# panbanda/islands

Measured on AMD Instinct MI355X. Metric: queries/sec @ recall@10>=0.95, 10Mx768 ef=128, higher is better.
Workload: dtype f32; 1 GPU; 10000000 x 768 f32 rows resident in HBM (in-memory provider), hierarchical Gaussian mixture, graph by the harness (tools/synth.py::build_graph: k-means medoid levels flattened into one layer, diversified links, parent->child and reverse edges), deg<= 60 (mean 38.6), query batch 1024, k=10, ef=128, cosine; nodes=10000000, dim=768, query_batch=1024, k=10, ef=128, graph=harness, distinct_leaves=False, parallelism=single, searches_in_flight=32, distinct_batches=497, replayed_queries=1688

## Files before the change

### include/islands_amd.h

```cpp
#ifndef ISLANDS_AMD_H
#define ISLANDS_AMD_H

#include <stddef.h>
#include <stdint.h>

#ifdef __cplusplus
extern "C" {
#endif

#define ISL_ABI_VERSION 3

typedef int32_t isl_status;

enum {
  ISL_OK = 0,
  ISL_ERR_DIMENSION_MISMATCH = 1,
  ISL_ERR_EMPTY_COLLECTION = 2,
  ISL_ERR_INVALID_CONFIG = 3,
  ISL_ERR_INDEX_NOT_BUILT = 4,
  ISL_ERR_NODE_NOT_FOUND = 5,
  ISL_ERR_SERIALIZATION = 6,
  ISL_ERR_DESERIALIZATION = 7,
  ISL_ERR_IO = 8,
  ISL_ERR_HNSW = 9,
// ... 76 lines not shown
                            uint64_t n_new, uint64_t d, const uint64_t* levels, int32_t mem, uint64_t* first_id);
#define ISL_REMOVED UINT64_MAX
#define ISL_REMOVE_MAX_CANDIDATES 512u
isl_status isl_index_remove(isl_index* idx, const isl_build_options* opts, const uint64_t* ids, uint64_t n_ids,
                            uint64_t* out_remap , uint64_t* out_len );
isl_status isl_select_neighbors(const isl_index* idx, const isl_build_options* opts,
                                const uint64_t* base_ids, uint64_t nb, const uint64_t* cand_ids,
                                uint64_t pitch, const uint32_t* cand_cnt, uint64_t cap,
                                uint64_t* out_ids, uint32_t* out_cnt);

isl_status isl_index_from_bytes(const uint8_t* bytes, size_t len, isl_index** out);
isl_status isl_index_to_bytes(const isl_index* idx, uint8_t** out, size_t* len);
void isl_free_bytes(uint8_t* p);
void isl_index_free(isl_index* idx);

typedef struct isl_index_metadata {
  uint32_t version;
  uint64_t num_vectors;
  uint64_t dimension;
  int64_t created_at;
  int64_t updated_at;
  int32_t has_description;
  char description[256];
} isl_index_metadata;
void isl_index_metadata_new(uint64_t num_vectors, uint64_t dimension, int64_t now, isl_index_metadata* out);
isl_status isl_storage_write_metadata(const isl_index_metadata* meta, uint8_t** out, size_t* len);
isl_status isl_storage_read_metadata(const uint8_t* bytes, size_t len, isl_index_metadata* meta,
                                     size_t* consumed);
isl_status isl_index_save(const isl_index* idx, const char* path, const isl_index_metadata* meta);
isl_status isl_index_load(const char* path, isl_index** out, isl_index_metadata* meta);

uint64_t isl_index_len(const isl_index* idx);
int32_t isl_index_is_empty(const isl_index* idx);
int32_t isl_index_dimension(const isl_index* idx, uint64_t* dim);
uint64_t isl_index_storage_bytes(const isl_index* idx);
int32_t isl_index_is_recompute(const isl_index* idx);
int32_t isl_index_is_compact(const isl_index* idx);
isl_status isl_index_config(const isl_index* idx, isl_leann_config* out);
int32_t isl_index_entry_point(const isl_index* idx, uint64_t* entry);
uint64_t isl_index_max_level(const isl_index* idx);
int32_t isl_index_get_neighbors(const isl_index* idx, uint64_t node, const uint64_t** ptr,
                                size_t* len);

isl_status isl_index_upload(isl_index* idx, int32_t device);

isl_status isl_set_embeddings(isl_index* idx, const void* rows, uint64_t n, uint64_t d,
                              int32_t dtype, int32_t mem);

typedef struct isl_search_stats {
  uint64_t queries;
  uint64_t expansions;
  uint64_t edges;
  uint64_t evals;
  uint64_t pushes;
  uint64_t exact_path;
  uint64_t replayed;
  double kernel_ms;
  uint64_t encoded_nodes;
  uint64_t recompute_rounds;
  uint64_t allocations;
} isl_search_stats;

isl_status isl_index_prepare(isl_index* idx, uint64_t max_nq, uint64_t max_ef, uint64_t max_k,
                             int32_t lanes);

isl_status isl_search_batch(const isl_index* idx, const float* queries, uint64_t nq, uint64_t d,
                            uint64_t k, uint64_t ef, uint64_t* out_ids, float* out_dist,
                            uint32_t* out_count);
isl_status isl_search_batch_async(const isl_index* idx, const float* queries, uint64_t nq, uint64_t d,
                                  uint64_t k, uint64_t ef, uint64_t* out_ids, float* out_dist,
                                  uint32_t* out_count, uint64_t* token);
isl_status isl_search_batch_device(const isl_index* idx, const float* d_queries, uint64_t nq,
                                   uint64_t d, uint64_t k, uint64_t ef, uint64_t* d_out_ids,
                                   float* d_out_dist, uint32_t* d_out_count, void* stream);
isl_status isl_search_batch_device_async(const isl_index* idx, const float* d_queries, uint64_t nq,
                                         uint64_t d, uint64_t k, uint64_t ef, uint64_t* d_out_ids,
                                         float* d_out_dist, uint32_t* d_out_count, void* stream,
                                         uint64_t* token);
isl_status isl_search_wait_stats(const isl_index* idx, uint64_t token, isl_search_stats* stats);
isl_status isl_search_wait(const isl_index* idx, uint64_t token);
isl_status isl_search_stream_wait(const isl_index* idx, uint64_t token, void* stream);
isl_status isl_index_group_counters(const isl_index* idx, uint64_t* launches, uint64_t* shared_launches,
                                    uint64_t* shared_calls);
isl_status isl_search(const isl_index* idx, const float* query, uint64_t d, uint64_t k,
                      uint64_t* out_ids, float* out_dist, uint32_t* out_count);

isl_status isl_search_last_stats(const isl_index* idx, isl_search_stats* out);

#define ISL_MAX_ENTRY_SEEDS 65536ull
isl_status isl_index_select_entry_seeds(isl_index* idx, uint64_t count, uint64_t* out_ids, uint64_t* out_count);
isl_status isl_index_set_entry_seeds(isl_index* idx, const uint64_t* ids, uint64_t count);
isl_status isl_index_entry_seeds(const isl_index* idx, uint64_t* out, uint64_t cap, uint64_t* count);
isl_status isl_index_pick_entries(const isl_index* idx, const float* queries, uint64_t nq, uint64_t d,
                                  uint64_t* out_ids, int32_t mem, void* stream);

isl_status isl_distance(int32_t metric, const float* a, uint64_t na, const float* b, uint64_t nb,
                        float* out);
isl_status isl_distance_squared(int32_t metric, const float* a, uint64_t na, const float* b,
                                uint64_t nb, float* out);
isl_status isl_distance_batch(int32_t metric, const float* query, uint64_t d, const float* rows,
                              uint64_t n, uint64_t row_len, float* out, int32_t mem, int32_t device,
                              void* stream);
isl_status isl_normalize_rows(float* rows, uint64_t n, uint64_t d, int32_t mem, int32_t device,
                              void* stream);

isl_status isl_distance_matrix(int32_t metric, const float* queries, uint64_t nq, const float* rows,
                               uint64_t n, uint64_t d, float* out, int32_t mem, int32_t device,
                               void* stream);
isl_status isl_bruteforce_topk(int32_t metric, const float* queries, uint64_t nq, const float* rows,
                               uint64_t n, uint64_t d, uint64_t k, uint64_t* out_ids, float* out_dist,
                               uint32_t* out_count, int32_t mem, int32_t device, void* stream);

isl_status isl_merge_topk(uint64_t nlists, uint64_t nq, uint64_t k, const uint64_t* ids,
                          const float* scores, const uint32_t* counts, const uint64_t* id_base,
                          uint64_t top_k, uint64_t* out_ids, float* out_scores,
                          uint32_t* out_src, uint32_t* out_count, int32_t mem, int32_t device,
                          void* stream);
#define ISL_SHARD_POISON_COUNT 0xFFFFFFFFu
uint64_t isl_shard_record_bytes(uint64_t nq, uint64_t k);
isl_status isl_merge_topk_packed_async(uint64_t nlists, uint64_t nq, uint64_t k, const void* d_records,
                                       uint64_t list_stride, const uint64_t* d_id_base, uint64_t top_k,
                                       uint64_t* d_out_ids, float* d_out_scores, uint32_t* d_out_src,
                                       uint32_t* d_out_count, uint32_t* d_flags, int32_t device, void* stream);
#define ISL_SHARD_UNIQUE_ID_BYTES 128
typedef struct isl_shard_group isl_shard_group;
typedef int32_t (*isl_shard_allgather_fn)(void* user, const void* send, void* recv, uint64_t bytes);
isl_status isl_shard_unique_id(uint8_t id[ISL_SHARD_UNIQUE_ID_BYTES]);
isl_status isl_shard_group_create(int32_t device, int32_t world, int32_t rank,
                                  const uint8_t id[ISL_SHARD_UNIQUE_ID_BYTES], isl_shard_group** out);
isl_status isl_shard_group_create_host(int32_t device, int32_t world, int32_t rank,
                                       isl_shard_allgather_fn allgather, void* user, isl_shard_group** out);
isl_status isl_shard_group_info(const isl_shard_group* grp, int32_t* world, int32_t* rank, int32_t* comm_ranks,
                                int32_t* is_rccl);
void isl_shard_group_free(isl_shard_group* grp);

typedef struct isl_sharded_searcher isl_sharded_searcher;
isl_status isl_sharded_searcher_new(const isl_index* shard, isl_shard_group* grp, uint64_t n_total,
                                    const uint64_t* id_base, int32_t depth, isl_sharded_searcher** out);
void isl_sharded_searcher_free(isl_sharded_searcher* s);
isl_status isl_sharded_prepare(isl_sharded_searcher* s, uint64_t max_nq, uint64_t max_k, uint64_t max_ef);
isl_status isl_sharded_submit(isl_sharded_searcher* s, const float* d_queries, uint64_t nq, uint64_t d,
                              uint64_t k, uint64_t ef, void* stream, uint64_t* handle);
isl_status isl_sharded_result(isl_sharded_searcher* s, uint64_t handle, const uint64_t** d_ids,
                              const float** d_dist, const uint32_t** d_src, const uint32_t** d_count,
                              isl_search_stats* stats);
isl_status isl_sharded_search_batch(isl_sharded_searcher* s, const float* queries, uint64_t nq, uint64_t d,
                                    uint64_t k, uint64_t ef, uint64_t* out_ids, float* out_dist,
                                    uint32_t* out_src, uint32_t* out_count);
isl_status isl_sharded_flags(isl_sharded_searcher* s, uint32_t* flags);

isl_status isl_merge_service(uint64_t nlists, uint64_t nq, uint64_t k, const uint64_t* ids,
                             const float* distances, const uint32_t* counts,
                             const uint64_t* files_len, uint64_t top_k, uint64_t* out_ids,
                             float* out_scores, uint32_t* out_src, uint32_t* out_count,
                             int32_t mem, int32_t device, void* stream);

typedef struct isl_pq isl_pq;
isl_status isl_pq_new(uint64_t dimension, uint64_t m, uint64_t K, const float* codebooks,
                      int32_t metric, int32_t device, isl_pq** out);
void isl_pq_free(isl_pq* pq);
isl_status isl_pq_build_distance_tables(const isl_pq* pq, const float* queries, uint64_t nq,
                                        uint64_t d, float* tables, int32_t mem, void* stream);
isl_status isl_pq_table_distance(const isl_pq* pq, const float* tables, const uint16_t* codes,
                                 uint64_t n, float* out, int32_t mem, void* stream);
isl_status isl_pq_asymmetric_distance(const isl_pq* pq, const float* query, uint64_t d,
                                      const uint16_t* codes, uint64_t n, float* out, int32_t mem,
// ... 109 lines not shown
```

### include/islands_amd.hpp

```cpp
#pragma once

#include <cstdint>
#include <optional>
#include <stdexcept>
#include <string>
#include <utility>
#include <vector>

#include "islands_amd.h"

namespace islands::core {

struct CoreError : std::runtime_error {
  isl_status status;
  uint64_t expected, actual, node;
  CoreError(isl_status s, const std::string& msg, uint64_t e = 0, uint64_t a = 0, uint64_t n = 0)
      : std::runtime_error(msg), status(s), expected(e), actual(a), node(n) {}
  std::string kind() const { return isl_status_name(status); }
};

inline void check(isl_status s) {
  if (s != ISL_OK)
    throw CoreError(s, isl_last_error_message(), isl_last_error_expected(),
                    isl_last_error_actual(), isl_last_error_node());
// ... 117 lines not shown
    uint64_t first = 0;
    check(isl_index_insert(h_, &opts, n ? vectors.data() : nullptr, ISL_DTYPE_F32, n, d, levels, ISL_MEM_HOST, &first));
    return first;
  }
  uint64_t insert_bf16(const std::vector<uint16_t>& rows_bits, uint64_t n, uint64_t d,
                       const isl_build_options& opts = build_options(), const uint64_t* levels = nullptr) {
    uint64_t first = 0;
    check(isl_index_insert(h_, &opts, n ? rows_bits.data() : nullptr, ISL_DTYPE_BF16, n, d, levels, ISL_MEM_HOST,
                           &first));
    return first;
  }
  std::vector<uint64_t> remove(const std::vector<uint64_t>& ids, const isl_build_options& opts = build_options()) {
    std::vector<uint64_t> remap(len());
    check(isl_index_remove(h_, &opts, ids.empty() ? nullptr : ids.data(), ids.size(), remap.data(), nullptr));
    return remap;
  }
  std::vector<uint64_t> select_neighbors(uint64_t base, const std::vector<uint64_t>& candidates, uint64_t cap,
                                         const isl_build_options& opts = build_options()) const {
    std::vector<uint64_t> out(cap ? cap : 1);
    uint32_t cnt = (uint32_t)candidates.size(), n = 0;
    check(isl_select_neighbors(h_, &opts, &base, 1, candidates.data(), candidates.size(), &cnt, cap, out.data(), &n));
    out.resize(n);
    return out;
  }
  std::vector<uint8_t> to_bytes() const {
    uint8_t* p = nullptr;
    size_t n = 0;
    check(isl_index_to_bytes(h_, &p, &n));
    std::vector<uint8_t> out(p, p + n);
    isl_free_bytes(p);
    return out;
  }
  LeannIndex(LeannIndex&& o) noexcept : h_(o.h_) { o.h_ = nullptr; }
  LeannIndex& operator=(LeannIndex&& o) noexcept {
    if (this != &o) { isl_index_free(h_); h_ = o.h_; o.h_ = nullptr; }
    return *this;
  }
  LeannIndex(const LeannIndex&) = delete;
  LeannIndex& operator=(const LeannIndex&) = delete;
  ~LeannIndex() { isl_index_free(h_); }

  uint64_t len() const { return isl_index_len(h_); }
  bool is_empty() const { return isl_index_is_empty(h_) != 0; }
  std::optional<uint64_t> dimension() const {
    uint64_t d = 0;
    return isl_index_dimension(h_, &d) ? std::optional<uint64_t>(d) : std::nullopt;
  }
  uint64_t storage_bytes() const { return isl_index_storage_bytes(h_); }
  bool is_recompute() const { return isl_index_is_recompute(h_) != 0; }
  bool is_compact() const { return isl_index_is_compact(h_) != 0; }
  LeannConfig config() const { LeannConfig c; check(isl_index_config(h_, &c)); return c; }

  void upload(int32_t device = 0) { check(isl_index_upload(h_, device)); }
  void attach(const InMemoryEmbeddingProvider& p) {
    check(isl_set_embeddings(h_, p.embeddings.data(), p.len(), p.dim, ISL_DTYPE_F32, ISL_MEM_HOST));
  }
  void attach_recompute(isl_encoder* enc, const std::vector<uint16_t>& tokens, uint64_t n, uint64_t L,
                        bool normalize = true, bool keep_rows = false) {
    check(isl_set_recompute_provider(h_, enc, tokens.data(), nullptr, n, L, normalize ? 1 : 0,
                                     keep_rows ? 1 : 0, ISL_MEM_HOST));
  }
  std::vector<uint64_t> select_entry_seeds(uint64_t count) {
    std::vector<uint64_t> ids(count < len() ? count : len());
    uint64_t n = 0;
    check(isl_index_select_entry_seeds(h_, count, ids.data(), &n));
    ids.resize(n);
    return ids;
  }
  void set_entry_seeds(const std::vector<uint64_t>& ids) { check(isl_index_set_entry_seeds(h_, ids.data(), ids.size())); }
  std::vector<uint64_t> entry_seeds() const {
    uint64_t n = 0;
    check(isl_index_entry_seeds(h_, nullptr, 0, &n));
    std::vector<uint64_t> ids(n);
    check(isl_index_entry_seeds(h_, ids.data(), n, &n));
    return ids;
  }
  std::vector<uint64_t> pick_entries(const std::vector<float>& queries, uint64_t nq) const {
    std::vector<uint64_t> ids(nq);
    check(isl_index_pick_entries(h_, queries.data(), nq, nq ? queries.size() / nq : 0, ids.data(), ISL_MEM_HOST, nullptr));
    return ids;
  }
  void prepare(uint64_t max_nq, uint64_t max_ef, uint64_t max_k = 10, int32_t lanes = 8) {
    check(isl_index_prepare(h_, max_nq, max_ef, max_k, lanes));
  }
  std::vector<std::pair<uint64_t, float>> search(const std::vector<float>& query, uint64_t k) const {
    return search_with_params(query, k, config().ef_search);
  }
  std::vector<std::pair<uint64_t, float>> search_with_params(const std::vector<float>& query,
                                                             uint64_t k, uint64_t ef) const {
    std::vector<uint64_t> ids(k ? k : 1);
    std::vector<float> dist(k ? k : 1);
    uint32_t cnt = 0;
    check(isl_search_batch(h_, query.data(), 1, query.size(), k, ef, ids.data(), dist.data(), &cnt));
    std::vector<std::pair<uint64_t, float>> out;
    for (uint32_t i = 0; i < cnt; i++) out.emplace_back(ids[i], dist[i]);
    return out;
  }
  void attach_pq_codes(const isl_pq* pq, const std::vector<uint16_t>& codes, uint64_t n) {
    check(isl_index_set_pq_codes(h_, pq, codes.data(), n, ISL_MEM_HOST));
  }
  std::vector<std::pair<uint64_t, float>> search_two_level(const std::vector<float>& query, uint64_t k,
                                                           uint64_t ef, float rerank_ratio) const {
    std::vector<uint64_t> ids(k ? k : 1);
    std::vector<float> dist(k ? k : 1);
    uint32_t cnt = 0;
    check(isl_search_two_level_batch(h_, query.data(), 1, query.size(), k, ef, rerank_ratio, ids.data(),
                                     dist.data(), &cnt));
    std::vector<std::pair<uint64_t, float>> out;
    for (uint32_t i = 0; i < cnt; i++) out.emplace_back(ids[i], dist[i]);
    return out;
  }
  isl_index* handle() const { return h_; }

 private:
  explicit LeannIndex(std::nullptr_t) {}
  isl_index* h_ = nullptr;
};

struct SearchResult {
  uint64_t id = 0;
  float score = 0.f;
  std::optional<std::vector<float>> vector;
  std::optional<std::string> text;
  float to_similarity() const { return 1.0f / (1.0f + score); }
};

struct SearchConfig {
  uint64_t top_k = 10, ef = 100;
  bool include_vectors = false, include_metadata = true;
  std::optional<float> min_similarity;
  static SearchConfig fast(uint64_t k) { SearchConfig c; c.top_k = k; c.ef = k * 2; return c; }
  static SearchConfig accurate(uint64_t k) { SearchConfig c; c.top_k = k; c.ef = k * 10; return c; }
};

class HnswGraph {
 public:
  HnswGraph(const std::vector<float>& vectors, uint64_t dim,
            const std::vector<std::vector<std::vector<uint64_t>>>& layers,
            const std::vector<uint64_t>& levels, std::optional<uint64_t> entry_point, uint64_t max_level,
            uint64_t m = 16, uint64_t m0 = 32, uint64_t ef_construction = 200,
            DistanceMetric metric = DistanceMetric::Cosine, int32_t device = 0)
      : vectors_(vectors), dim_(dim) {
    const uint64_t n = levels.size();
    std::vector<std::vector<uint64_t>> offs(layers.size()), adjs(layers.size());
    std::vector<const uint64_t*> po, pa;
    for (size_t L = 0; L < layers.size(); L++) {
      offs[L].assign(1, 0);
      for (uint64_t i = 0; i < n; i++) {
        adjs[L].insert(adjs[L].end(), layers[L][i].begin(), layers[L][i].end());
        offs[L].push_back(adjs[L].size());
      }
      if (adjs[L].empty()) adjs[L].push_back(0);
      po.push_back(offs[L].data());
      pa.push_back(adjs[L].data());
    }
    check(isl_hnsw_from_layers(m, m0, ef_construction, (int32_t)metric, n, dim, layers.size(), po.data(),
                               pa.data(), n ? levels.data() : nullptr, entry_point ? 1 : 0,
                               entry_point.value_or(0), max_level, n ? vectors.data() : nullptr, device, &h_));
  }
  static HnswGraph from_bytes(const std::vector<uint8_t>& bytes, int32_t device = 0) {
    HnswGraph g;
    check(isl_hnsw_from_bytes(bytes.data(), bytes.size(), device, &g.h_));
    return g;
  }
  static HnswGraph build(const std::vector<float>& vectors, uint64_t dim, const isl_hnsw_config* cfg = nullptr,
                         const std::vector<uint64_t>& levels = {}, uint64_t level_seed = 0,
// ... 176 lines not shown
```

### islands_amd/__init__.py

```python
from __future__ import annotations

import ctypes as C
import enum
import os
from dataclasses import dataclass, field

import numpy as np

from . import _ffi
from ._ffi import BertConfigC, BuildOptionsC, IndexMetadataC, LeannConfigC, SearchStatsC, u64

__all__ = [
    "CoreError", "DistanceMetric", "PruningStrategy", "LeannConfig", "CsrGraph",
    "InMemoryEmbeddingProvider", "LeannIndex", "ProductQuantizer", "SearchResult",
    "batch_calculate", "calculate", "calculate_squared", "normalize_rows", "distance_matrix",
    "bruteforce_topk", "merge_topk", "merge_service",
    "device_count", "HnswGraph", "SearchConfig", "Searcher", "MultiIndexSearcher",
    "mean_pool_normalize", "service_search", "BertConfig", "CandleEmbedder", "IndexMetadata",
]

MEM_HOST, MEM_DEVICE = 0, 1
SELECT_REFERENCE, SELECT_DIVERSE = 0, 1
_SELECT_RULES = {"reference": SELECT_REFERENCE, "diverse": SELECT_DIVERSE}
REMOVED = 0xFFFFFFFFFFFFFFFF
# ... 618 lines not shown
            q = q.reshape(1, -1)
        nq, d = q.shape
        ids = np.zeros((nq, max(k, 1)), dtype=np.uint64)
        dist = np.zeros((nq, max(k, 1)), dtype=np.float32)
        cnt = np.zeros(nq, dtype=np.uint32)
        _check(_ffi.lib().isl_search_two_level_batch(self._h, _ptr(q), nq, d, k, ef,
                                                     C.c_float(rerank_ratio), _ptr(ids), _ptr(dist),
                                                     _ptr(cnt)))
        return ids[:, :k], dist[:, :k], cnt

    def search_two_level_batch_device(self, d_queries_ptr: int, nq: int, d: int, k: int, ef: int,
                                      rerank_ratio: float, d_ids_ptr: int, d_dist_ptr: int,
                                      d_count_ptr: int, stream: int = 0):
        _check(_ffi.lib().isl_search_two_level_batch_device(
            self._h, C.c_void_p(d_queries_ptr), nq, d, k, ef, C.c_float(rerank_ratio),
            C.c_void_p(d_ids_ptr), C.c_void_p(d_dist_ptr), C.c_void_p(d_count_ptr),
            C.c_void_p(stream)))

    def search_two_level_batch_device_async(self, d_queries_ptr: int, nq: int, d: int, k: int, ef: int,
                                            rerank_ratio: float, d_ids_ptr: int, d_dist_ptr: int,
                                            d_count_ptr: int, stream: int = 0) -> int:
        tok = C.c_uint64()
        _check(_ffi.lib().isl_search_two_level_batch_device_async(
            self._h, C.c_void_p(d_queries_ptr), nq, d, k, ef, C.c_float(rerank_ratio),
            C.c_void_p(d_ids_ptr), C.c_void_p(d_dist_ptr), C.c_void_p(d_count_ptr),
            C.c_void_p(stream), C.byref(tok)))
        return int(tok.value)

    def search_batch_device(self, d_queries_ptr: int, nq: int, d: int, k: int, ef: int,
                            d_ids_ptr: int, d_dist_ptr: int, d_count_ptr: int, stream: int = 0):
        _check(_ffi.lib().isl_search_batch_device(
            self._h, C.c_void_p(d_queries_ptr), nq, d, k, ef, C.c_void_p(d_ids_ptr),
            C.c_void_p(d_dist_ptr), C.c_void_p(d_count_ptr), C.c_void_p(stream)))

    def search_batch_device_async(self, d_queries_ptr: int, nq: int, d: int, k: int, ef: int,
                                  d_ids_ptr: int, d_dist_ptr: int, d_count_ptr: int,
                                  stream: int = 0) -> int:
        tok = C.c_uint64()
        _check(_ffi.lib().isl_search_batch_device_async(
            self._h, C.c_void_p(d_queries_ptr), nq, d, k, ef, C.c_void_p(d_ids_ptr),
            C.c_void_p(d_dist_ptr), C.c_void_p(d_count_ptr), C.c_void_p(stream), C.byref(tok)))
        return int(tok.value)

    def wait(self, token: int):
        try:
            _check(_ffi.lib().isl_search_wait(self._h, token))
        finally:
            out = self._pending.pop(token, None)
        return out

    def wait_stats(self, token: int) -> dict:
        s = SearchStatsC()
        try:
            _check(_ffi.lib().isl_search_wait_stats(self._h, token, C.byref(s)))
        finally:
            self._pending.pop(token, None)
        return {f: getattr(s, f) for f, _ in SearchStatsC._fields_}

    def prepare(self, max_nq: int, max_ef: int, max_k: int = 10, lanes: int = 8) -> "LeannIndex":
        _check(_ffi.lib().isl_index_prepare(self._h, max_nq, max_ef, max_k, lanes))
        return self

    def search_batch_async(self, queries, k: int, ef: int, out=None) -> int:
        q = _f32(queries)
        if q.ndim == 1:
            q = q.reshape(1, -1)
        nq, d = q.shape
        if out is None:
            out = (np.zeros((nq, max(k, 1)), dtype=np.uint64), np.zeros((nq, max(k, 1)), dtype=np.float32),
                   np.zeros(nq, dtype=np.uint32))
        ids, dist, cnt = out
        tok = C.c_uint64()
        _check(_ffi.lib().isl_search_batch_async(self._h, _ptr(q), nq, d, k, ef, _ptr(ids), _ptr(dist),
                                                 _ptr(cnt), C.byref(tok)))
        t = int(tok.value)
        if t:
            self._pending[t] = out
        return t

    def last_stats(self) -> dict:
        s = SearchStatsC()
        _check(_ffi.lib().isl_search_last_stats(self._h, C.byref(s)))
        return {f: getattr(s, f) for f, _ in SearchStatsC._fields_}


def merge_topk(ids, scores, counts, top_k: int, id_base=None, device: int = 0):
    ids = np.ascontiguousarray(ids, dtype=np.uint64)
    scores = _f32(scores)
    counts = np.ascontiguousarray(counts, dtype=np.uint32)
    nl, nq, k = ids.shape
    base = None if id_base is None else np.ascontiguousarray(id_base, dtype=np.uint64)
    oi = np.zeros((nq, max(top_k, 1)), dtype=np.uint64)
    osc = np.zeros((nq, max(top_k, 1)), dtype=np.float32)
    osrc = np.zeros((nq, max(top_k, 1)), dtype=np.uint32)
    oc = np.zeros(nq, dtype=np.uint32)
    _check(_ffi.lib().isl_merge_topk(nl, nq, k, _ptr(ids), _ptr(scores), _ptr(counts),
                                     None if base is None else _ptr(base), top_k, _ptr(oi),
                                     _ptr(osc), _ptr(osrc), _ptr(oc), MEM_HOST, device, None))
    return oi[:, :top_k], osc[:, :top_k], osrc[:, :top_k], oc


def merge_service(ids, distances, counts, top_k: int, files_len=None, device: int = 0):
    ids = np.ascontiguousarray(ids, dtype=np.uint64)
    distances = _f32(distances)
    counts = np.ascontiguousarray(counts, dtype=np.uint32)
    nl, nq, k = ids.shape
    fl = None if files_len is None else np.ascontiguousarray(files_len, dtype=np.uint64)
    oi = np.zeros((nq, max(top_k, 1)), dtype=np.uint64)
    osc = np.zeros((nq, max(top_k, 1)), dtype=np.float32)
    osrc = np.zeros((nq, max(top_k, 1)), dtype=np.uint32)
    oc = np.zeros(nq, dtype=np.uint32)
    _check(_ffi.lib().isl_merge_service(nl, nq, k, _ptr(ids), _ptr(distances), _ptr(counts),
                                        None if fl is None else _ptr(fl), top_k, _ptr(oi),
                                        _ptr(osc), _ptr(osrc), _ptr(oc), MEM_HOST, device, None))
    return oi[:, :top_k], osc[:, :top_k], osrc[:, :top_k], oc


class ProductQuantizer:

    def __init__(self, dimension: int, codebooks, metric=DistanceMetric.Euclidean, device: int = 0):
        cb = _f32(codebooks)
        m, K, dsub = cb.shape
        if m * dsub != dimension:
            raise CoreError(3, f"Invalid configuration: dimension {dimension} must be divisible by "
                               f"num_subquantizers {m}")
        self.dimension, self.m, self.K, self.dsub = dimension, m, K, dsub
        self._h = C.c_void_p()
        _check(_ffi.lib().isl_pq_new(dimension, m, K, _ptr(cb), int(metric), device,
                                     C.byref(self._h)))

    def __del__(self):
        h = getattr(self, "_h", None)
        if h:
            try:
                _ffi.lib().isl_pq_free(h)
            except Exception:
                pass
            self._h = None

    def num_subquantizers(self) -> int:
        return self.m

    def bytes_per_vector(self) -> int:
        return self.m if self.K <= 256 else self.m * 2

    def compression_ratio(self) -> float:
        return float(np.float32(self.dimension * 4) / np.float32(self.bytes_per_vector()))

    def build_distance_tables(self, queries) -> np.ndarray:
        q = _f32(queries)
        single = q.ndim == 1
        if single:
            q = q.reshape(1, -1)
        nq, d = q.shape
        t = np.zeros((nq, self.m, self.K), dtype=np.float32)
        _check(_ffi.lib().isl_pq_build_distance_tables(self._h, _ptr(q), nq, d, _ptr(t), MEM_HOST,
                                                       None))
        return t[0] if single else t

    def table_distance(self, tables, codes) -> np.ndarray:
        t = _f32(tables)
        c = np.ascontiguousarray(codes, dtype=np.uint16).reshape(-1, self.m)
        out = np.zeros(c.shape[0], dtype=np.float32)
        _check(_ffi.lib().isl_pq_table_distance(self._h, _ptr(t), _ptr(c), c.shape[0], _ptr(out),
                                                MEM_HOST, None))
        return out
# ... 487 lines not shown
```

### islands_amd/_ffi.py

```python
from __future__ import annotations

import ctypes as C
import os

os.environ.setdefault("GPU_MAX_HW_QUEUES", "32")

_HERE = os.path.dirname(os.path.abspath(__file__))
LIB_PATH = os.environ.get("ISL_AMD_LIB") or os.path.join(_HERE, "lib", "libislands_amd.so")

u64, u32, i32, f32 = C.c_uint64, C.c_uint32, C.c_int32, C.c_float
P = C.POINTER


class LeannConfigC(C.Structure):
    _fields_ = [
        ("m", u64), ("m0", u64), ("ef_construction", u64), ("ml", C.c_double),
        ("max_layers", u64), ("metric", u32), ("ef_search", u64), ("beam_width", u64),
        ("prune_ratio", f32), ("pruning_strategy", u32), ("high_degree_pruning", C.c_uint8),
        ("hub_percentile", f32), ("is_compact", C.c_uint8), ("is_recompute", C.c_uint8),
    ]


class BertConfigC(C.Structure):
    _fields_ = [("vocab_size", u32), ("hidden", u32), ("layers", u32), ("heads", u32),
                ("intermediate", u32), ("max_position", u32), ("type_vocab", u32),
                ("layer_norm_eps", f32), ("gelu_tanh", u32)]


class IndexMetadataC(C.Structure):
    _fields_ = [("version", u32), ("num_vectors", u64), ("dimension", u64), ("created_at", C.c_int64),
                ("updated_at", C.c_int64), ("has_description", i32), ("description", C.c_char * 256)]


class SearchStatsC(C.Structure):
    _fields_ = [("queries", u64), ("expansions", u64), ("edges", u64), ("evals", u64),
                ("pushes", u64), ("exact_path", u64), ("replayed", u64), ("kernel_ms", C.c_double),
                ("encoded_nodes", u64), ("recompute_rounds", u64), ("allocations", u64)]


class BuildOptionsC(C.Structure):
    _fields_ = [("struct_size", u32), ("select_rule", u32), ("alpha", f32), ("keep_pruned", u32),
                ("batch", u64)]


class HnswConfigC(C.Structure):
    _fields_ = [("m", u64), ("m0", u64), ("ef_construction", u64), ("ml", C.c_double), ("metric", u32),
                ("max_layers", u64)]


SIGNATURES = {
    "isl_last_error_message": (C.c_char_p, []),
    "isl_last_error_expected": (u64, []),
    "isl_last_error_actual": (u64, []),
    "isl_last_error_node": (u64, []),
    "isl_status_name": (C.c_char_p, [i32]),
    "isl_abi_version": (u32, []),
    "isl_device_count": (i32, []),
    "isl_leann_config_paper_default": (None, [P(LeannConfigC)]),
    "isl_leann_config_fast": (None, [P(LeannConfigC)]),
    "isl_leann_config_accurate": (None, [P(LeannConfigC)]),
    "isl_leann_config_validate": (i32, [P(LeannConfigC)]),
    "isl_index_new": (i32, [P(LeannConfigC), P(C.c_void_p)]),
    "isl_index_from_csr": (i32, [P(LeannConfigC), u64, C.c_void_p, C.c_void_p, C.c_void_p,
                                 C.c_void_p, i32, u64, u64, i32, u64, P(C.c_void_p)]),
    "isl_index_from_device_csr": (i32, [P(LeannConfigC), i32, u64, C.c_void_p, C.c_void_p, i32,
                                        u64, i32, u64, P(C.c_void_p)]),
    "isl_index_from_bytes": (i32, [C.c_void_p, C.c_size_t, P(C.c_void_p)]),
    "isl_index_to_bytes": (i32, [C.c_void_p, P(C.c_void_p), P(C.c_size_t)]),
    "isl_free_bytes": (None, [C.c_void_p]),
    "isl_index_free": (None, [C.c_void_p]),
    "isl_index_len": (u64, [C.c_void_p]),
    "isl_index_is_empty": (i32, [C.c_void_p]),
    "isl_index_dimension": (i32, [C.c_void_p, P(u64)]),
    "isl_index_storage_bytes": (u64, [C.c_void_p]),
    "isl_index_is_recompute": (i32, [C.c_void_p]),
    "isl_index_is_compact": (i32, [C.c_void_p]),
    "isl_index_config": (i32, [C.c_void_p, P(LeannConfigC)]),
    "isl_index_entry_point": (i32, [C.c_void_p, P(u64)]),
    "isl_index_max_level": (u64, [C.c_void_p]),
    "isl_index_get_neighbors": (i32, [C.c_void_p, u64, P(P(u64)), P(C.c_size_t)]),
    "isl_index_upload": (i32, [C.c_void_p, i32]),
    "isl_set_embeddings": (i32, [C.c_void_p, C.c_void_p, u64, u64, i32, i32]),
    "isl_search_batch": (i32, [C.c_void_p, C.c_void_p, u64, u64, u64, u64, C.c_void_p,
                               C.c_void_p, C.c_void_p]),
    "isl_hnsw_from_bytes": (i32, [C.c_void_p, C.c_size_t, i32, P(C.c_void_p)]),
    "isl_distance_matrix_bf16": (i32, [i32, C.c_void_p, u64, C.c_void_p, u64, u64, C.c_void_p, i32, i32,
                                       C.c_void_p]),
    "isl_index_set_pq_codes": (i32, [C.c_void_p, C.c_void_p, C.c_void_p, u64, i32]),
    "isl_search_two_level_batch": (i32, [C.c_void_p, C.c_void_p, u64, u64, u64, u64, C.c_float,
                                         C.c_void_p, C.c_void_p, C.c_void_p]),
    "isl_search_two_level_batch_device": (i32, [C.c_void_p, C.c_void_p, u64, u64, u64, u64,
                                                C.c_float, C.c_void_p, C.c_void_p, C.c_void_p,
                                                C.c_void_p]),
    "isl_search_two_level_batch_device_async": (i32, [C.c_void_p, C.c_void_p, u64, u64, u64, u64,
                                                      C.c_float, C.c_void_p, C.c_void_p, C.c_void_p,
                                                      C.c_void_p, P(u64)]),
    "isl_search_batch_device": (i32, [C.c_void_p, C.c_void_p, u64, u64, u64, u64, C.c_void_p,
                                      C.c_void_p, C.c_void_p, C.c_void_p]),
    "isl_search_batch_device_async": (i32, [C.c_void_p, C.c_void_p, u64, u64, u64, u64, C.c_void_p,
                                            C.c_void_p, C.c_void_p, C.c_void_p, P(u64)]),
    "isl_search_wait": (i32, [C.c_void_p, u64]),
    "isl_search_stream_wait": (i32, [C.c_void_p, u64, C.c_void_p]),
    "isl_index_group_counters": (i32, [C.c_void_p, P(u64), P(u64), P(u64)]),
    "isl_shard_record_bytes": (u64, [u64, u64]),
    "isl_merge_topk_packed_async": (i32, [u64, u64, u64, C.c_void_p, u64, C.c_void_p, u64, C.c_void_p, C.c_void_p,
                                          C.c_void_p, C.c_void_p, C.c_void_p, i32, C.c_void_p]),
    "isl_shard_unique_id": (i32, [C.c_void_p]),
    "isl_shard_group_create": (i32, [i32, i32, i32, C.c_void_p, P(C.c_void_p)]),
    "isl_shard_group_create_host": (i32, [i32, i32, i32, C.c_void_p, C.c_void_p, P(C.c_void_p)]),
    "isl_shard_group_info": (i32, [C.c_void_p, P(i32), P(i32), P(i32), P(i32)]),
    "isl_shard_group_free": (None, [C.c_void_p]),
    "isl_sharded_searcher_new": (i32, [C.c_void_p, C.c_void_p, u64, C.c_void_p, i32, P(C.c_void_p)]),
    "isl_sharded_searcher_free": (None, [C.c_void_p]),
    "isl_sharded_prepare": (i32, [C.c_void_p, u64, u64, u64]),
    "isl_sharded_submit": (i32, [C.c_void_p, C.c_void_p, u64, u64, u64, u64, C.c_void_p, P(u64)]),
    "isl_sharded_result": (i32, [C.c_void_p, u64, P(C.c_void_p), P(C.c_void_p), P(C.c_void_p), P(C.c_void_p),
                                 P(SearchStatsC)]),
    "isl_sharded_search_batch": (i32, [C.c_void_p, C.c_void_p, u64, u64, u64, u64, C.c_void_p, C.c_void_p,
                                       C.c_void_p, C.c_void_p]),
    "isl_sharded_flags": (i32, [C.c_void_p, P(u32)]),
    "isl_search_wait_stats": (i32, [C.c_void_p, u64, P(SearchStatsC)]),
    "isl_search_batch_async": (i32, [C.c_void_p, C.c_void_p, u64, u64, u64, u64, C.c_void_p,
                                     C.c_void_p, C.c_void_p, P(u64)]),
    "isl_index_prepare": (i32, [C.c_void_p, u64, u64, u64, i32]),
    "isl_search": (i32, [C.c_void_p, C.c_void_p, u64, u64, C.c_void_p, C.c_void_p, C.c_void_p]),
    "isl_search_last_stats": (i32, [C.c_void_p, P(SearchStatsC)]),
    "isl_distance": (i32, [i32, C.c_void_p, u64, C.c_void_p, u64, P(f32)]),
    "isl_distance_squared": (i32, [i32, C.c_void_p, u64, C.c_void_p, u64, P(f32)]),
    "isl_distance_batch": (i32, [i32, C.c_void_p, u64, C.c_void_p, u64, u64, C.c_void_p, i32, i32,
                                 C.c_void_p]),
    "isl_normalize_rows": (i32, [C.c_void_p, u64, u64, i32, i32, C.c_void_p]),
    "isl_distance_matrix": (i32, [i32, C.c_void_p, u64, C.c_void_p, u64, u64, C.c_void_p, i32, i32,
                                  C.c_void_p]),
    "isl_bruteforce_topk": (i32, [i32, C.c_void_p, u64, C.c_void_p, u64, u64, u64, C.c_void_p,
                                  C.c_void_p, C.c_void_p, i32, i32, C.c_void_p]),
    "isl_row_sumsq_bf16": (i32, [C.c_void_p, u64, u64, C.c_void_p, i32, i32, C.c_void_p]),
    "isl_distance_matrix_bf16_norms": (i32, [i32, C.c_void_p, u64, C.c_void_p, u64, u64, C.c_void_p, C.c_void_p,
                                             C.c_void_p, i32, i32, C.c_void_p]),
    "isl_distance_matrix_bf16_enqueue": (i32, [i32, C.c_void_p, u64, C.c_void_p, u64, u64, C.c_void_p, C.c_void_p,
                                               C.c_void_p, i32, C.c_void_p]),
    "isl_bruteforce_topk_bf16": (i32, [i32, C.c_void_p, u64, C.c_void_p, u64, u64, u64, C.c_void_p,
                                       C.c_void_p, C.c_void_p, i32, i32, C.c_void_p]),
    "isl_merge_topk": (i32, [u64, u64, u64, C.c_void_p, C.c_void_p, C.c_void_p, C.c_void_p, u64,
                             C.c_void_p, C.c_void_p, C.c_void_p, C.c_void_p, i32, i32,
                             C.c_void_p]),
    "isl_merge_service": (i32, [u64, u64, u64, C.c_void_p, C.c_void_p, C.c_void_p, C.c_void_p, u64,
                             C.c_void_p, C.c_void_p, C.c_void_p, C.c_void_p, i32, i32,
                             C.c_void_p]),
    "isl_index_build": (i32, [P(LeannConfigC), C.c_void_p, u64, u64, C.c_void_p, u64, i32, i32,
                              P(C.c_void_p)]),
    "isl_build_options_default": (None, [P(BuildOptionsC)]),
    "isl_index_build_ex": (i32, [P(LeannConfigC), P(BuildOptionsC), C.c_void_p, u64, u64, C.c_void_p, i32, i32,
                                 P(C.c_void_p)]),
    "isl_index_build_rows": (i32, [P(LeannConfigC), P(BuildOptionsC), C.c_void_p, i32, u64, u64, C.c_void_p, i32, i32,
                                   P(C.c_void_p)]),
    "isl_select_neighbors": (i32, [C.c_void_p, P(BuildOptionsC), C.c_void_p, u64, C.c_void_p, u64, C.c_void_p,
                                   u64, C.c_void_p, C.c_void_p]),
    "isl_index_select_entry_seeds": (i32, [C.c_void_p, u64, C.c_void_p, P(u64)]),
    "isl_index_set_entry_seeds": (i32, [C.c_void_p, C.c_void_p, u64]),
    "isl_index_entry_seeds": (i32, [C.c_void_p, C.c_void_p, u64, P(u64)]),
    "isl_index_pick_entries": (i32, [C.c_void_p, C.c_void_p, u64, u64, C.c_void_p, i32, C.c_void_p]),
    "isl_index_metadata_new": (None, [u64, u64, C.c_int64, P(IndexMetadataC)]),
    "isl_storage_write_metadata": (i32, [P(IndexMetadataC), P(C.c_void_p), P(C.c_size_t)]),
    "isl_storage_read_metadata": (i32, [C.c_void_p, C.c_size_t, P(IndexMetadataC), P(C.c_size_t)]),
    "isl_index_save": (i32, [C.c_void_p, C.c_char_p, P(IndexMetadataC)]),
    "isl_index_load": (i32, [C.c_char_p, P(C.c_void_p), P(IndexMetadataC)]),
    "isl_encoder_new": (i32, [P(BertConfigC), i32, P(C.c_void_p)]),
    "isl_encoder_free": (None, [C.c_void_p]),
    "isl_encoder_set_weight": (i32, [C.c_void_p, C.c_char_p, C.c_void_p, u64, i32]),
    "isl_encoder_set_precision": (i32, [C.c_void_p, i32]),
    "isl_encoder_forward": (i32, [C.c_void_p, C.c_void_p, C.c_void_p, C.c_void_p, u64, u64,
                                  C.c_void_p, i32, C.c_void_p]),
    "isl_encoder_embed": (i32, [C.c_void_p, C.c_void_p, C.c_void_p, C.c_void_p, u64, u64, i32,
                                C.c_void_p, i32, C.c_void_p]),
    "isl_set_recompute_provider": (i32, [C.c_void_p, C.c_void_p, C.c_void_p, C.c_void_p, u64, u64,
                                         i32, i32, i32]),
    "isl_index_set_recompute_cache_rows": (i32, [C.c_void_p, u64]),
    "isl_index_recompute_cache_bytes": (u64, [C.c_void_p]),
    "isl_mean_pool_normalize": (i32, [C.c_void_p, C.c_void_p, u64, u64, u64, i32, C.c_void_p, i32,
                                      i32, C.c_void_p]),
    "isl_hnsw_from_layers": (i32, [u64, u64, u64, i32, u64, u64, u64, C.c_void_p, C.c_void_p,
                                   C.c_void_p, i32, u64, u64, C.c_void_p, i32, P(C.c_void_p)]),
    "isl_hnsw_free": (None, [C.c_void_p]),
    "isl_hnsw_len": (u64, [C.c_void_p]),
    "isl_hnsw_last_stats": (i32, [C.c_void_p, P(SearchStatsC)]),
    "isl_hnsw_search_batch": (i32, [C.c_void_p, C.c_void_p, u64, u64, u64, u64, C.c_void_p,
# ... 49 lines not shown
```

### islands_amd/csrc/common.hpp

```cpp
#pragma once

#include <hip/hip_runtime.h>

#include <algorithm>
#include <cstdarg>
#include <cstdint>
#include <cstdlib>
#include <cstdio>
#include <cstring>
#include <atomic>
#include <chrono>
#include <mutex>
#include <string>
#include <thread>
#include <type_traits>
#include <vector>

#include "../../include/islands_amd.h"
#include "device_buffer.hpp"
#include "row_table.hpp"

namespace isl {

struct ErrorRecord {
  std::string message;
  uint64_t expected = 0, actual = 0, node = 0;
};
ErrorRecord& last_error();
isl_status fail(isl_status st, const char* fmt, ...);
isl_status fail_dim(uint64_t expected, uint64_t actual);
isl_status fail_node(uint64_t node);

#define ISL_HIP(expr)                                                                   \
  do {                                                                                  \
    hipError_t _e = (expr);                                                             \
    if (_e != hipSuccess)                                                               \
      return ::isl::fail(ISL_ERR_DEVICE, "%s failed: %s (%s:%d)", #expr,                \
                         hipGetErrorString(_e), __FILE__, __LINE__);                    \
  } while (0)

#define ISL_TRY(expr)            \
  do {                           \
    isl_status _s = (expr);      \
    if (_s != ISL_OK) return _s; \
  } while (0)

template <class F>
void by_metric(uint32_t metric, F&& f) {
  switch (metric) {
    case ISL_METRIC_COSINE: f(std::integral_constant<int, ISL_METRIC_COSINE>{}); break;
    case ISL_METRIC_EUCLIDEAN: f(std::integral_constant<int, ISL_METRIC_EUCLIDEAN>{}); break;
    case ISL_METRIC_DOT: f(std::integral_constant<int, ISL_METRIC_DOT>{}); break;
    default: f(std::integral_constant<int, ISL_METRIC_MANHATTAN>{}); break;
  }
}

isl_status use_device(int32_t device);
int device_cu_count(int32_t device);

struct SearchWorkspace {
  uint32_t slots = 0;
  uint32_t ovf_bits = 0;
  DeviceBuffer<uint32_t> ovf_tab;
  DeviceBuffer<uint32_t> status;
  DeviceBuffer<uint64_t> payload;
  DeviceBuffer<uint32_t> ctr;
  DeviceBuffer<uint32_t> ticket;
  DeviceBuffer<uint32_t> redo;
  DeviceBuffer<uint32_t> replay;
  DeviceBuffer<uint32_t> qsel;
  DeviceBuffer<uint32_t> qsel_h;
  DeviceBuffer<uint64_t> plog;
  DeviceBuffer<float> q_stage;
  DeviceBuffer<uint64_t> ids_stage;
  DeviceBuffer<float> dist_stage;
  DeviceBuffer<uint32_t> count_stage;
  PinnedBuffer<float> h_q;
  PinnedBuffer<uint64_t> h_ids;
  PinnedBuffer<float> h_dist;
  PinnedBuffer<uint32_t> h_count;
  hipStream_t stream = nullptr;
  hipEvent_t ev0 = nullptr, ev1 = nullptr, ev_in = nullptr, ev_done = nullptr;
  bool busy = false;
  bool waiting = false;
  bool enqueued = false;
  bool ticket_clean = false;
  bool publish_results = false;
  uint64_t token = 0;
  uint64_t nq_inflight = 0, k_inflight = 0;
  uint32_t ef_inflight = 0;
  bool fast_inflight = false;
  hipStream_t st_inflight = nullptr;
  uint64_t* u_ids = nullptr;
  float* u_dist = nullptr;
  uint32_t* u_count = nullptr;
  PinnedBuffer<uint32_t> h_status;
  PinnedBuffer<uint32_t> h_ctr;
  PinnedBuffer<uint32_t> h_head;
  DeviceBuffer<uint64_t> d_prof;
  DeviceBuffer<uint64_t> d_tline;
  DeviceBuffer<uint32_t> q_entry;
  DeviceBuffer<float> co_q;
  DeviceBuffer<uint64_t> co_ids;
  DeviceBuffer<float> co_dist;
  DeviceBuffer<uint32_t> co_cnt;
  DeviceBuffer<uint32_t> miss;
  DeviceBuffer<uint32_t> uniq;
  DeviceBuffer<uint32_t> uniq_count;
  uint64_t miss_cap = 0;
  uint64_t pref_cap = 0;
  DeviceBuffer<uint32_t> qstate;
  DeviceBuffer<uint32_t> qflag;
  DeviceBuffer<uint32_t> qlist;
  PinnedBuffer<uint32_t> h_qlist;
  DeviceBuffer<uint32_t> uslots;
  DeviceBuffer<uint32_t> xslot;
  PinnedBuffer<uint32_t> h_xlist;
  DeviceBuffer<float> tl_tables;
  std::thread* worker = nullptr;
  bool threaded = false;
  isl_status worker_status = ISL_OK;
  ErrorRecord worker_error;
  uint64_t alloc_events = 0;
  uint64_t alloc_mark = 0;
  isl_search_stats stats{};
  bool grp = false;
  SearchWorkspace* grp_launch = nullptr;
  uint32_t grp_offset = 0;
  hipEvent_t grp_ready = nullptr;
  uint64_t grp_allocs = 0;
  bool grp_failed = false;
  isl_status grp_status = ISL_OK;
  ErrorRecord grp_error;
  int32_t pool_lane = -1;
  bool union_launch = false;
  PinnedBuffer<uint64_t> h_members;
  DeviceBuffer<uint32_t> grp_scratch;
};

constexpr int kSearchLanes = 32;

int hw_queues_at_load();
constexpr int kGroupBelowQueues = 8;
struct GroupSwitches { bool off; uint32_t cap, room; };
inline GroupSwitches group_switches() {
  auto num = [](const char* name) -> uint32_t {
    const char* e = getenv(name);
    const long long v = e ? atoll(e) : 0;
    return v > 0 ? (uint32_t)std::min<long long>(v, 0x7FFFFFFF) : 0u;
  };
  const char* off = getenv("ISL_NO_GROUP");
  const bool is_off = (off && *off) ? strcmp(off, "0") != 0 : hw_queues_at_load() >= kGroupBelowQueues;
  return GroupSwitches{is_off, num("ISL_GROUP_CAP"), num("ISL_GROUP_ROOM")};
}
struct GroupState;

struct ExactPool {
  uint32_t slots = 0;
  uint64_t cand_cap = 0;
  DeviceBuffer<float> cand_d;
  DeviceBuffer<uint32_t> cand_id;
  DeviceBuffer<uint32_t> vis_bits;
  uint64_t vis_words = 0;
  DeviceBuffer<uint32_t> ulist;
  uint32_t ulist_cap = 0;
  DeviceBuffer<uint32_t> locks;
  DeviceBuffer<uint32_t> xstate;
  uint32_t xstate_words = 0;
};

}

struct isl_pq {
  uint64_t dimension = 0, m = 0, K = 0, dsub = 0, cstride = 0;
  int32_t metric = ISL_METRIC_EUCLIDEAN;
  int32_t device = 0;
  isl::DeviceBuffer<float> d_codebooks;
};

struct isl_index {
  isl_leann_config cfg{};
  bool host_csr_valid = true;
  std::vector<uint64_t> node_offsets{0};
  std::vector<uint64_t> neighbors;
  std::vector<uint64_t> levels;
  std::vector<uint64_t> degree_counts;
  bool has_entry = false;
  uint64_t entry_point = 0;
  uint64_t max_level = 0;
  uint64_t num_nodes = 0;
  bool has_dimension = false;
  uint64_t dimension = 0;

  int32_t device = -1;
  isl::DeviceBuffer<uint64_t> d_off;
  isl::DeviceBuffer<uint32_t> d_adj;
  uint64_t nnz = 0;
  uint32_t max_degree = 0;
  mutable std::atomic<uint64_t> evals_hint{0};
  isl::RowTable rows;
  uint64_t nvec = 0;

  isl::EntrySeeds seeds;

  uint32_t* d_ell = nullptr;
  uint32_t* d_ell_deg = nullptr;
  uint32_t ell_w = 0;
  isl::DeviceBuffer<uint32_t> ell_copy, ell_deg_copy;

  uint32_t* build_q_entry = nullptr;
  uint32_t* build_q_evals = nullptr;

  struct isl_encoder* enc = nullptr;
  isl::DeviceBuffer<uint16_t> d_tokens;
  isl::DeviceBuffer<uint16_t> d_lens;
  uint32_t tok_L = 0;
  isl::DeviceBuffer<uint32_t> d_slot_of;
  isl::DeviceBuffer<uint32_t> d_owner;
  isl::DeviceBuffer<uint32_t> d_stamp;
  isl::DeviceBuffer<uint32_t> d_slab_head;
  mutable uint32_t round_no = 1;
  bool recompute = false, keep_rows = false;
  int32_t enc_normalize = 1;

  bool is_hnsw = false;
  uint64_t hnsw_layers = 0;
  isl::DeviceBuffer<const uint64_t*> d_layer_off;
  isl::DeviceBuffer<const uint32_t*> d_layer_adj;
  std::vector<isl::DeviceBuffer<unsigned char>> hnsw_owned;

  const isl_pq* pq = nullptr;
  isl::DeviceBuffer<uint16_t> d_codes;
  uint64_t ncodes = 0;

  mutable std::mutex mu;
  mutable std::mutex recompute_mu;
  struct RecJoin {
    std::mutex mu;
    std::mutex leader;
    std::vector<void*> waiting;
  };
  mutable RecJoin rec_join;
  mutable isl::SearchWorkspace ws[isl::kSearchLanes];
  mutable isl::ExactPool pool;
  mutable uint64_t next_token = 1;
  const isl::GroupSwitches group_sw = isl::group_switches();
  mutable std::mutex group_mu;
  mutable isl::GroupState* group = nullptr;
};

struct isl_hnsw {
  isl_index* core = nullptr;
  uint64_t m = 0, m0 = 0, ef_construction = 0;
  uint64_t dim = 0;
  double ml = 0.0;
  uint64_t max_layers = 16;
  int32_t device = 0;
  std::vector<const uint64_t*> layer_off;
  std::vector<const uint32_t*> layer_adj;
  mutable std::mutex host_mu;
  mutable bool host_valid = false;
  mutable std::vector<std::vector<uint64_t>> h_off;
  mutable std::vector<std::vector<uint64_t>> h_adj;
};

namespace isl {
isl_status search_device_sync(const isl_index* idx, const float* d_queries, uint64_t nq, uint64_t d,
                              uint64_t k, uint64_t ef, uint64_t* d_ids, float* d_dist,
                              uint32_t* d_count, hipStream_t stream);
isl_status poison_failed_queries(const isl_index* idx, uint64_t token, uint32_t* d_counts, uint64_t nq, hipStream_t stream);
isl_status materialise_host_csr(const isl_index* idx);
isl_status set_grown_embeddings(isl_index* idx, const isl_index* old, const void* rows, int32_t dtype, uint64_t n_new,
                                uint64_t d, int32_t mem);
isl_status pq_launch_tables(const isl_pq* pq, const float* d_queries, uint64_t nq, float* d_tables,
                            hipStream_t st);
isl_status launch_entry_pick(const isl_index* idx, const float* d_queries, uint64_t nq, uint32_t* q_entry,
                             uint32_t* q_evals, unsigned long long* packed, uint32_t* status, uint64_t* d_out_ids,
                             hipStream_t st);
isl_status env_entry_seeds(isl_index* idx);
void free_workspace(SearchWorkspace& ws);
void free_exact_pool(ExactPool& pool);
bool any_lane_busy(const isl_index* idx);
void join_lane_workers(const isl_index* idx);
void free_group_state(isl_index* idx);
isl_status ensure_padded_adjacency(isl_index* idx);
isl_status hnsw_config_validate(uint64_t m, uint64_t m0, uint64_t ef_construction, int64_t metric);
isl_status attach_upper_layers(isl_hnsw* h, const std::vector<const uint64_t*>& offs,
                               const std::vector<const uint32_t*>& adjs);
}
```

### islands_amd/csrc/search.hip

```cpp
#include "search_geometry.hpp"
#include "search_internal.hpp"

using namespace isl_lane;

namespace {

__global__ void fill_u32_kernel(uint32_t* p, uint64_t n, uint32_t v) {
  uint64_t i = (uint64_t)blockIdx.x * blockDim.x + threadIdx.x;
  uint64_t stride = (uint64_t)gridDim.x * blockDim.x;
  for (; i < n; i += stride) p[i] = v;
}

struct PublishParams {
  const uint32_t* src[6];
  uint32_t* dst[6];
  uint32_t words[6];
  uint32_t ticket_seg;
};
__global__ void publish_kernel(PublishParams pp) {
  const uint32_t seg = blockIdx.y;
  const uint32_t n = pp.words[seg];
  const uint32_t* __restrict__ src = pp.src[seg];
  uint32_t* __restrict__ dst = pp.dst[seg];
  for (uint32_t i = blockIdx.x * blockDim.x + threadIdx.x; i < n; i += gridDim.x * blockDim.x) {
    dst[i] = src[i];
    if (seg == pp.ticket_seg) const_cast<uint32_t*>(src)[i] = 0u;
  }
}
__global__ void copy_u128_kernel(const uint4* __restrict__ src, uint4* __restrict__ dst, uint64_t n) {
  for (uint64_t i = (uint64_t)blockIdx.x * blockDim.x + threadIdx.x; i < n; i += (uint64_t)gridDim.x * blockDim.x)
    dst[i] = src[i];
}
__global__ void copy_u32_kernel(const uint32_t* __restrict__ src, uint32_t* __restrict__ dst, uint64_t n) {
  for (uint64_t i = (uint64_t)blockIdx.x * blockDim.x + threadIdx.x; i < n; i += (uint64_t)gridDim.x * blockDim.x)
    dst[i] = src[i];
}

__global__ void seed_redo_kernel(const uint32_t* __restrict__ list, uint32_t n, uint32_t* __restrict__ redo,
                                 uint32_t* __restrict__ ticket) {
  for (uint32_t i = threadIdx.x; i < n; i += blockDim.x) redo[i] = list[i];
  if (threadIdx.x == 0) ticket[1] = n;
}

constexpr uint32_t kExactSlots = 32;
constexpr uint32_t kOvfBits = 15;


hipStream_t pool_stream(int32_t device, uint32_t lane, bool* created) {
  static std::mutex mu;
  static hipStream_t pool[64][32];
  static const uint32_t size = [] {
    const char* e = getenv("ISL_MAX_STREAMS");
    const int v = e ? atoi(e) : 16;
    return (uint32_t)std::min(std::max(v, 1), 32);
  }();
  *created = false;
  if (device < 0 || device >= 64) return nullptr;
  std::lock_guard<std::mutex> lock(mu);
  hipStream_t& st = pool[device][lane % size];
  if (!st) {
    if (hipStreamCreateWithFlags(&st, hipStreamNonBlocking) != hipSuccess) { (void)hipGetLastError(); st = nullptr; }
    else *created = true;
  }
  return st;
}

}

isl_status isl_lane::ensure_lane_stream(const isl_index* idx, isl::SearchWorkspace& ws) {
  if (ws.stream) return ISL_OK;
  bool created = false;
  hipStream_t st = pool_stream(idx->device, ws.pool_lane >= 0 ? (uint32_t)ws.pool_lane : (uint32_t)(&ws - idx->ws), &created);
  if (!st) return isl::fail(ISL_ERR_DEVICE, "hipStreamCreate failed for a search lane");
  if (created) ws.alloc_events++;
  if (!ws.ev_done) { ISL_HIP(hipEventCreateWithFlags(&ws.ev_done, hipEventDisableTiming)); ws.alloc_events++; }
  if (!ws.ev0) { ISL_HIP(hipEventCreate(&ws.ev0)); ws.alloc_events++; }
  if (!ws.ev1) { ISL_HIP(hipEventCreate(&ws.ev1)); ws.alloc_events++; }
  if (!ws.ev_in) { ISL_HIP(hipEventCreateWithFlags(&ws.ev_in, hipEventDisableTiming)); ws.alloc_events++; }
  if (!ws.ticket) {
    ISL_TRY(ws.ticket.reserve(16, &ws.alloc_events));
    ws.ticket_clean = false;
  }
  ISL_TRY(ws.h_head.reserve(16, &ws.alloc_events));
  ws.stream = st;
  return ISL_OK;
}

void isl_lane::copy_words(const uint32_t* src, uint32_t* dst, uint64_t n, uint32_t grid, uint32_t block, hipStream_t st) {
  hipLaunchKernelGGL(copy_u32_kernel, dim3(grid), dim3(block), 0, st, src, dst, n);
}

isl_status isl_lane::prepare_workspace(const isl_index* idx, isl::SearchWorkspace& ws, uint32_t nq, uint32_t slots,
                                       uint32_t plog_cap) {
  ISL_TRY(ensure_lane_stream(idx, ws));
  uint64_t* const ev = &ws.alloc_events;
  const uint64_t cap = nq < 1024 ? 1024 : nq;
  ISL_TRY(ws.h_status.reserve(cap, ev));
  ISL_TRY(ws.h_ctr.reserve(cap * 4, ev));
  if (ws.slots < slots || !ws.ovf_tab) {
    ws.ovf_tab.reset();
    ws.slots = 0;
    static const uint32_t ovf_bits_cfg = [] {
      const char* e = getenv("ISL_OVF_BITS");
      const int v = e ? atoi(e) : (int)kOvfBits;
      return (uint32_t)std::min(15, std::max(10, v));
    }();
    ws.ovf_bits = ovf_bits_cfg;
    uint64_t n = (uint64_t)slots << ovf_bits_cfg;
    ISL_TRY(ws.ovf_tab.reserve(n, ev));
    hipLaunchKernelGGL(fill_u32_kernel, dim3(2048), dim3(256), 0, ws.stream, ws.ovf_tab, n, EMPTY);
    ISL_HIP(hipGetLastError());
    ISL_HIP(hipStreamSynchronize(ws.stream));
    ws.slots = slots;
  }
  ISL_TRY(ws.status.reserve(cap, ev));
  ISL_TRY(ws.payload.reserve(cap, ev));
  ISL_TRY(ws.ctr.reserve(cap * 4, ev));
  ISL_TRY(ws.redo.reserve(cap, ev));
  ISL_TRY(ws.replay.reserve(cap, ev));
  ISL_TRY(ws.qsel.reserve(cap, ev));
  ISL_TRY(ws.qsel_h.reserve(cap, ev));
  return ws.plog.reserve(ws.status.capacity() * plog_cap, ev);
}

namespace {

isl_status prepare_host_staging(isl::SearchWorkspace& ws, uint64_t nq, uint64_t d, uint64_t k) {
  uint64_t* const ev = &ws.alloc_events;
  ISL_TRY(ws.q_stage.reserve(nq * d, ev));
  ISL_TRY(ws.h_q.reserve(nq * d, ev));
  const uint64_t slots = nq * std::max<uint64_t>(k, 1);
  ISL_TRY(ws.ids_stage.reserve(slots, ev));
  ISL_TRY(ws.dist_stage.reserve(slots, ev));
  ISL_TRY(ws.count_stage.reserve(slots, ev));
  ISL_TRY(ws.h_ids.reserve(slots, ev));
  ISL_TRY(ws.h_dist.reserve(slots, ev));
  return ws.h_count.reserve(slots, ev);
}

}

isl_status isl_lane::ensure_pool(const isl_index* idx, isl::SearchWorkspace& ws) {
  isl::ExactPool& pl = idx->pool;
  if (pl.slots) return ISL_OK;
  uint64_t max_id = std::max(idx->num_nodes, idx->nvec);
  pl.vis_words = (max_id + 31) / 32 + 1;
  pl.cand_cap = std::min<uint64_t>(max_id + 1, 1ull << 21);
  pl.ulist_cap = std::max<uint32_t>(idx->max_degree, 64);
  isl_status st = ISL_OK;
  uint64_t* const ev = &ws.alloc_events;
  pl.xstate_words = 16 + 2 * (kMaxExactEf + 1);
  if ((st = pl.cand_d.reserve(kExactSlots * pl.cand_cap, ev)) == ISL_OK &&
      (st = pl.cand_id.reserve(kExactSlots * pl.cand_cap, ev)) == ISL_OK &&
      (st = pl.vis_bits.reserve(kExactSlots * pl.vis_words, ev)) == ISL_OK &&
      (st = pl.ulist.reserve((uint64_t)kExactSlots * pl.ulist_cap, ev)) == ISL_OK &&
      (st = pl.locks.reserve(kExactSlots, ev)) == ISL_OK &&
      (st = pl.xstate.reserve((uint64_t)kExactSlots * pl.xstate_words, ev)) == ISL_OK) {
    if (hipMemset(pl.locks, 0, (size_t)kExactSlots * 4) == hipSuccess) {
      pl.slots = kExactSlots;
      return ISL_OK;
    }
    st = isl::fail(ISL_ERR_DEVICE, "hipMemset failed for the exact-kernel pool");
  }
  isl::free_exact_pool(pl);
  return st;
}

namespace {

__global__ void pad_rows_kernel(const uint64_t* __restrict__ off, const uint32_t* __restrict__ adj, uint64_t n,
                                uint32_t W, uint32_t* __restrict__ ell, uint32_t* __restrict__ deg) {
  const uint64_t row = (uint64_t)blockIdx.x * 4 + (threadIdx.x >> 6);
  const uint32_t lane = threadIdx.x & 63;
  if (row >= n) return;
  const uint64_t o0 = off[row];
  const uint32_t d = (uint32_t)(off[row + 1] - o0);
  for (uint32_t i = lane; i < W; i += 64) ell[row * W + i] = i < d ? adj[o0 + i] : EMPTY;
  if (lane == 0) deg[row] = d;
}

isl_status publish(isl::SearchWorkspace& ws, uint64_t nq, uint64_t k, hipStream_t st) {
  PublishParams pp{};
  uint32_t n = 0;
  auto seg = [&](const void* src, void* dst, uint64_t words) {
    pp.src[n] = (const uint32_t*)src; pp.dst[n] = (uint32_t*)dst; pp.words[n] = (uint32_t)words; ++n;
  };
  seg(ws.status, ws.h_status, nq);
  seg(ws.ctr, ws.h_ctr, nq * 4);
  pp.ticket_seg = n;
  seg(ws.ticket, ws.h_head, 16);
  if (ws.publish_results) {
    seg(ws.count_stage, ws.h_count, nq);
    if (k) {
      seg(ws.ids_stage, ws.h_ids, nq * k * 2);
      seg(ws.dist_stage, ws.h_dist, nq * k);
    }
  }
  hipLaunchKernelGGL(publish_kernel, dim3(16, n), dim3(256), 0, st, pp);
  ISL_HIP(hipGetLastError());
  ws.ticket_clean = true;
  return ISL_OK;
}


void launch_fast(const isl_launch::FastKernel& k, uint32_t grid, size_t lds, hipStream_t st, const SearchParams& p) {
  switch (k.S) {
    case 1: isl_launch::launch_fast_segments<1>(k, grid, lds, st, &p); break;
    case 2: isl_launch::launch_fast_segments<2>(k, grid, lds, st, &p); break;
    case 4: isl_launch::launch_fast_segments<4>(k, grid, lds, st, &p); break;
    default: isl_launch::launch_fast_segments<8>(k, grid, lds, st, &p); break;
  }
}

isl_status search_enqueue_impl(const isl_index* idx, isl::SearchWorkspace& ws, const SearchCall& c,
                               const RoundPlan& plan, bool warm) {
  const uint64_t nq = c.nq, d = c.d, k = c.k;
  if (nq > 0x7FFFFFFFull) return isl::fail(ISL_ERR_INVALID_ARGUMENT, "too many queries");
  const TwoLevelCall tl_call{c.ratio, plan.window_scale};
  const TwoLevelCall* tl = c.two_level ? &tl_call : nullptr;
  CallGeometry cg;
  ISL_TRY(call_geometry(idx, d, k, c.ef, tl, cg));
  const uint32_t ef = cg.ef;
  const bool use_fast = cg.use_fast;
  const bool resume = !warm && (plan.active != 0 || plan.exact != 0);
  const bool tl_qh = tl && !warm && !resume && idx->rows.is_bf16() && plan.retry == 0 && cg.tl_hbits_q == cg.fg.hbits;
  const bool qh = cg.qh && !resume;
  if (!warm)
    ISL_TRY(prepare_workspace(idx, ws, (uint32_t)nq,
                              (uint32_t)(idx->recompute ? nq : std::min<uint64_t>(nq, cg.lane_slots)), cg.plog_cap));
  if (!idx->pool.slots || ((use_fast || (tl && idx->max_degree <= 128)) && !idx->d_ell && idx->d_off && idx->num_nodes)) {
    std::lock_guard<std::mutex> lock(idx->mu);
    ISL_TRY(ensure_pool(idx, ws));
    const uint32_t* before = idx->d_ell;
    ISL_TRY(isl::ensure_padded_adjacency(const_cast<isl_index*>(idx)));
    if (idx->d_ell != before) ws.alloc_events += 2;
  }
  hipStream_t st = call_stream(ws, c);
  if (c.mode == StreamMode::OWN_AFTER_USER || c.mode == StreamMode::OWN_AFTER_EVENT) {
    if (c.mode == StreamMode::OWN_AFTER_USER) ISL_HIP(hipEventRecord(ws.ev_in, c.user_stream));
    ISL_HIP(hipStreamWaitEvent(ws.stream, ws.ev_in, 0));
  }

  SearchParams p{};
  p.off = idx->d_off;
  p.adj = idx->d_ell ? idx->d_ell : idx->d_adj;
  p.ell_w = idx->d_ell ? idx->ell_w : 0u;
  p.ell_deg = idx->d_ell_deg;
  p.num_nodes = idx->num_nodes;
  p.emb = idx->rows.data();
  p.emb_bf16 = idx->rows.is_bf16() ? 1u : 0u;
  p.norm2 = idx->rows.norm2();
  p.nvec = idx->nvec;
  p.stride = idx->rows.stride();
  p.d = (uint32_t)d;
  p.queries = c.queries;
  p.nq = warm ? 0u : (uint32_t)nq;
  p.k = (uint32_t)k;
  p.ef = ef;
  p.prune_ratio = idx->cfg.prune_ratio;
  p.prune_strategy = idx->cfg.pruning_strategy;
  p.entry = (uint32_t)std::min<uint64_t>(idx->entry_point, 0x7FFFFFF0ull);
  p.out_ids = c.ids;
  p.out_dist = c.dist;
  p.out_count = c.count;
  p.status = ws.status;
  p.payload = ws.payload;
  p.ctr = ws.ctr;
  p.ticket = ws.ticket;
  p.redo = ws.redo;
  ws.d_prof.reset();
  static const bool debug_env = getenv("ISL_DEBUG") != nullptr;
  if (debug_env && !warm) {
    ISL_TRY(ws.d_prof.reserve(nq * 8));
    ISL_HIP(hipMemset(ws.d_prof, 0, nq * 64));
  }
  p.prof = ws.d_prof;
  static const char* tline_env = getenv("ISL_TIMELINE");
  ws.d_tline.reset();
  if (tline_env && !warm) {
    ISL_TRY(ws.d_tline.reserve(nq * 2));
    ISL_HIP(hipMemset(ws.d_tline, 0, nq * 16));
  }
  p.tline = ws.d_tline;
  p.replay = ws.replay;
  p.plog = reinterpret_cast<uint2*>(ws.plog.get());
  p.plog_cap = cg.plog_cap;
  p.hbits = cg.fg.hbits;
  p.hcap = cg.fg.hcap;
  p.otab = ws.ovf_tab;
  p.obits = ws.ovf_bits;
  p.cand_d = idx->pool.cand_d;
  p.cand_id = idx->pool.cand_id;
  p.cand_cap = idx->pool.cand_cap;
  p.vis_bits = idx->pool.vis_bits;
  p.vis_words = idx->pool.vis_words;
  p.ulist = idx->pool.ulist;
  p.ulist_cap = idx->pool.ulist_cap;
  p.pool_locks = idx->pool.locks;
  p.pool_slots = idx->pool.slots;
  if (resume && !tl && plan.exact_parks) {
    p.xslot = ws.xslot;
    p.xstate = idx->pool.xstate;
    p.xstate_words = idx->pool.xstate_words;
  }
  p.slot_of = idx->recompute ? idx->d_slot_of : nullptr;
  p.stamp = idx->d_stamp;
  p.round_no = idx->round_no;
  if (resume) {
    p.qstate = ws.qstate;
    p.qstate_words = cg.state_words;
    p.qflag = ws.qflag;
    p.qlist = plan.listed ? ws.qlist : nullptr;
  } else if (tl && plan.retry) {
    p.qlist = ws.qlist;
  }
  p.miss = ws.miss;
  p.miss_cap = (uint32_t)std::min<uint64_t>(ws.miss_cap, 0xFFFFFFFFull);
  p.pref = ws.miss ? ws.miss + ws.miss_cap : nullptr;
  p.pref_cap = (uint32_t)ws.pref_cap;
  p.tl_prefetch = (tl && resume && ws.pref_cap) ? plan.prefetch : 0u;
  p.layer_off = idx->d_layer_off;
  p.layer_adj = idx->d_layer_adj;
  p.max_level = idx->is_hnsw ? (uint32_t)idx->max_level : 0u;
  p.hnsw_order = idx->is_hnsw ? 1u : 0u;
  p.q_entry = nullptr;
  p.q_evals = nullptr;
  if (idx->build_q_entry && !warm) {
    p.q_entry = idx->build_q_entry;
    p.q_evals = idx->build_q_evals;
    p.entry_given = 1u;
    p.max_level = 0u;
    ISL_HIP(hipMemsetAsync(ws.status, 0, nq * 4, st));
  }
  const bool seeded = idx->seeds.count() != 0 && !tl && !idx->recompute && !idx->is_hnsw && !idx->build_q_entry &&
                      !warm && !resume && nq != 0;
  if (seeded) {
    ISL_TRY(ws.q_entry.reserve(nq * 4, &ws.alloc_events));
    p.q_entry = ws.q_entry;
    p.q_evals = ws.q_entry + nq;
    p.entry_given = 1u;
    p.max_level = 0u;
  }
  if (tl) {
    const isl_pq* pq = idx->pq;
    const uint64_t want = std::max<uint64_t>(nq, 1) * pq->m * pq->K;
    ISL_TRY(ws.tl_tables.reserve(want, &ws.alloc_events));
    p.tl_tables = ws.tl_tables;
    p.tl_codes = idx->d_codes;
    p.tl_ncodes = idx->ncodes;
    p.tl_m = (uint32_t)pq->m;
    p.tl_K = (uint32_t)pq->K;
    p.tl_ratio = tl->ratio;
    p.tl_wcap = cg.tl_wcap;
  }
  const uint64_t nq_grid = warm ? 1 : nq;
  const int metric = (int)idx->cfg.metric;

  if (!ws.ticket_clean) ISL_HIP(hipMemsetAsync(ws.ticket, 0, 64, st));
  ws.ticket_clean = false;
  ISL_HIP(hipEventRecord(ws.ev0, st));
  if (resume && !tl && plan.exact) {
    hipLaunchKernelGGL(seed_redo_kernel, dim3(1), dim3(256), 0, st, ws.h_xlist, plan.exact, ws.redo, ws.ticket);
    ISL_HIP(hipGetLastError());
  }
  if (tl) {
    if (!warm && !plan.tables_built) ISL_TRY(isl::pq_launch_tables(idx->pq, c.queries, nq, ws.tl_tables, st));
    const uint64_t n_run = resume ? plan.active : plan.retry ? plan.retry : nq_grid;
    const uint32_t grid = (uint32_t)std::min<uint64_t>(n_run, cg.slots);
    p.nq = warm ? 0u : (uint32_t)n_run;
    if (tl_qh) {
      p.qsel = ws.qsel;
      p.qsel_h = ws.qsel_h;
      isl_launch::launch_classify((uint32_t)std::min<uint64_t>(nq_grid, 2048), st, &p);
      ISL_HIP(hipGetLastError());
      isl_launch::launch_two_level(metric, true, false, true, (uint32_t)std::min<uint64_t>(nq_grid, cg.tl_slots_q),
                                   cg.tl_lds_q, st, &p);
      ISL_HIP(hipGetLastError());
      p.qsel_mode = 1;
      isl_launch::launch_two_level(metric, true, false, false, grid, cg.tl_lds, st, &p);
      p.qsel_mode = 0;
    } else {
      isl_launch::launch_two_level(metric, p.emb_bf16 != 0, resume || (warm && idx->recompute), false, grid, cg.tl_lds, st, &p);
    }
    ISL_HIP(hipGetLastError());
    p.nq = warm ? 0u : (uint32_t)nq;
  } else
  if (use_fast && idx->is_hnsw && p.max_level > 0) {
    ISL_TRY(ws.q_entry.reserve(std::max<uint64_t>(nq, 1) * 2, &ws.alloc_events));
    p.q_entry = ws.q_entry;
    p.q_evals = ws.q_entry + nq;
    const uint32_t dgrid = (uint32_t)std::min<uint64_t>(nq_grid, 8192);
    isl_launch::launch_descent(metric, dgrid, cg.descent_lds, st, &p);
    ISL_HIP(hipGetLastError());
  }
  if (seeded) {
    ISL_TRY(isl::launch_entry_pick(idx, c.queries, nq, ws.q_entry, ws.q_entry + nq,
                                   reinterpret_cast<unsigned long long*>(ws.q_entry + 2 * nq), ws.status, nullptr, st));
  }
  if (tl) {
  } else if (use_fast) {
    if (resume) p.nq = plan.active;
    uint32_t grid = (uint32_t)std::min<uint64_t>(resume ? plan.active : nq_grid, cg.slots);
    const bool skip_fast = resume && plan.active == 0;
    isl_launch::FastKernel fk{cg.segments, metric, idx->max_degree > 64, p.emb_bf16 != 0, resume, false};
    if (qh) {
      p.qsel = ws.qsel;
      p.qsel_h = ws.qsel_h;
      isl_launch::launch_classify((uint32_t)std::min<uint64_t>(nq_grid, 2048), st, &p);
      ISL_HIP(hipGetLastError());
      p.hbits = cg.fgq.hbits;
      p.hcap = cg.fgq.hcap;
      fk.qh = true;
      launch_fast(fk, (uint32_t)std::min<uint64_t>(nq_grid, cg.slots_q), cg.fgq.lds, st, p);
      ISL_HIP(hipGetLastError());
      p.hbits = cg.fg.hbits;
      p.hcap = cg.fg.hcap;
      p.qsel_mode = 1;
      fk.qh = false;
      launch_fast(fk, grid, cg.fg.lds, st, p);
      p.qsel_mode = 0;
    } else if (!skip_fast) {
      launch_fast(fk, grid, cg.fg.lds, st, p);
    }
    ISL_HIP(hipGetLastError());
    p.nq = (uint32_t)nq;
  } else if (!warm && !resume) {
    std::vector<uint32_t> all(nq);
    for (uint64_t i = 0; i < nq; i++) all[i] = (uint32_t)i;
    uint32_t head0[4] = {0, (uint32_t)nq, 0, 0};
    ISL_HIP(hipMemcpyAsync(ws.redo, all.data(), nq * 4, hipMemcpyHostToDevice, st));
    ISL_HIP(hipMemcpyAsync(ws.ticket, head0, 16, hipMemcpyHostToDevice, st));
    ISL_HIP(hipStreamSynchronize(st));
  }
  if (!tl) {
    uint32_t grid = (uint32_t)std::min<uint64_t>(nq_grid, idx->pool.slots);
    isl_launch::launch_exact(metric, idx->is_hnsw, grid, cg.exact_lds, st, &p);
    ISL_HIP(hipGetLastError());
  }
  ISL_HIP(hipEventRecord(ws.ev1, st));
  ws.st_inflight = st;
  if (warm) return ISL_OK;

  if (!ws.union_launch) {
    ISL_TRY(publish(ws, nq, k, st));
    ISL_HIP(hipEventRecord(ws.ev_done, st));
  }
  ws.enqueued = true;
  ws.nq_inflight = nq;
  ws.k_inflight = k;
  ws.ef_inflight = ef;
  ws.fast_inflight = use_fast;
  return ISL_OK;
}

struct LastStats { const isl_index* idx = nullptr; isl_search_stats st{}; };
thread_local LastStats tl_last_stats;
void note_last_stats(const isl_index* idx, const isl_search_stats& st) {
  tl_last_stats.idx = idx;
  tl_last_stats.st = st;
}

}

isl_status isl_lane::search_enqueue(const isl_index* idx, isl::SearchWorkspace& ws, const SearchCall& c,
                                      const RoundPlan& plan, bool warm) {
  const isl_status st = search_enqueue_impl(idx, ws, c, plan, warm);
  if (st != ISL_OK) {
    const isl::ErrorRecord keep = isl::last_error();
    hipStream_t s = call_stream(ws, c);
    if (c.mode == StreamMode::USER || s) (void)hipStreamSynchronize(s);
    (void)hipGetLastError();
    ws.ticket_clean = false;
    ws.enqueued = false;
    isl::last_error() = keep;
  }
  return st;
}

isl_status isl_lane::search_finish(const isl_index* idx, isl::SearchWorkspace& ws, uint32_t* misses,
                                     bool defer_statuses) {
  if (!ws.enqueued) return isl::fail(ISL_ERR_INVALID_ARGUMENT, "no search in flight for this token");
  ws.enqueued = false;
  const uint64_t nq = ws.nq_inflight;
  const bool use_fast = ws.fast_inflight;
  const isl::SearchWorkspace& lw = ws.grp_launch ? *ws.grp_launch : ws;
  ISL_HIP(hipEventSynchronize(lw.ev_done));
  const uint32_t* status = ws.h_status;
  const uint32_t* ctr = ws.h_ctr;
  const uint32_t* head = ws.h_head;
  isl::DeviceBuffer<uint64_t> d_prof = std::move(ws.d_prof);
  float ms = 0.0f;
  (void)hipEventElapsedTime(&ms, lw.ev0, lw.ev1);

  isl_search_stats& ss = ws.stats;
  ss = isl_search_stats{};
  ss.queries = nq;
  ss.exact_path = head[1];
  ss.replayed = head[3];
  ss.kernel_ms = ms;
  ss.allocations = ws.alloc_events - ws.alloc_mark + ws.grp_allocs;
  for (uint64_t i = 0; i < nq; i++) {
    ss.expansions += ctr[i * 4 + 0];
    ss.edges += ctr[i * 4 + 1];
    ss.evals += ctr[i * 4 + 2];
    ss.pushes += ctr[i * 4 + 3];
  }
  if (use_fast && !idx->recompute && !misses && nq >= 16)
    idx->evals_hint.store(((uint64_t)ws.ef_inflight << 32) | std::min<uint64_t>(ss.evals / nq, 0xFFFFFFFFull),
                          std::memory_order_relaxed);
  if (ws.d_tline) {
    std::vector<uint64_t> tl(nq * 2 + 2);
    tl[0] = 0x154C494E45ull;
    tl[1] = nq;
    ISL_HIP(hipMemcpy(tl.data() + 2, ws.d_tline, nq * 16, hipMemcpyDeviceToHost));
    ws.d_tline.reset();
    static std::mutex tl_mu;
    std::lock_guard<std::mutex> lock(tl_mu);
    if (FILE* f = fopen(getenv("ISL_TIMELINE"), "ab")) {
      fwrite(tl.data(), 8, tl.size(), f);
      fclose(f);
    }
  }
  if (d_prof) {
    std::vector<uint64_t> pr(nq * 8);
    ISL_HIP(hipMemcpy(pr.data(), d_prof, nq * 64, hipMemcpyDeviceToHost));
    double sum[4] = {0, 0, 0, 0}, grp = 0, hr = 0;
    for (uint64_t i = 0; i < nq; i++) {
      for (int j = 0; j < 4; j++) sum[j] += pr[i * 8 + j] / 100.0;
      grp += pr[i * 8 + 4];
      hr += pr[i * 8 + 5];
    }
    fprintf(stderr, "[isl] per query: %.1f hops with new rows, %.1f distance passes of <= 16 rows\n", hr / nq,
            grp / nq);
    fprintf(stderr, "[isl] mean us per query by phase: select+adjacency %.0f, visited %.0f, rows+distance %.0f, "
            "insert %.0f\n", sum[0] / nq, sum[1] / nq, sum[2] / nq, sum[3] / nq);
  }
  if (getenv("ISL_DEBUG")) {
    std::vector<uint64_t> pay(nq);
    ISL_HIP(hipMemcpy(pay.data(), ws.payload, nq * 8, hipMemcpyDeviceToHost));
    std::vector<double> us;
    std::vector<std::pair<double, uint32_t>> byq;
    for (uint64_t i = 0; i < nq; i++)
      if (status[i] == QS_OK && pay[i]) { us.push_back(pay[i] / 100.0); byq.push_back({pay[i] / 100.0, ctr[i * 4]}); }
    std::sort(us.begin(), us.end());
    std::sort(byq.begin(), byq.end());
    if (!us.empty())
      fprintf(stderr, "[isl] per-query time in fast kernel (us): min %.0f p50 %.0f p90 %.0f p99 %.0f max %.0f; "
              "hops of slowest %u, of median %u; kernel %.0f us\n", us.front(), us[us.size() / 2],
              us[us.size() * 9 / 10], us[us.size() * 99 / 100], us.back(), byq.back().second,
              byq[byq.size() / 2].second, ms * 1000.0);
  }
  if (getenv("ISL_DEBUG") && (head[1] || head[3])) {
    fprintf(stderr, "[isl] %u of %llu queries re-run by the exact kernel (fast kernel %s): "
            "long-row %u, visited-overflow %u, tie-candidate overflow %u, push-log overflow %u, "
            "NaN/-0 distance %u; %u re-ordered by the replay kernel\n", head[1], (unsigned long long)nq,
            use_fast ? "on" : "off", head[9], head[10], head[11], head[8], head[12], head[3]);
  }
  if (misses) {
    *misses = head[13];
    if (head[13]) return ISL_OK;
  }
  if (defer_statuses) return ISL_OK;
  return search_statuses(ws, nq);
}

isl_status isl_lane::search_statuses(isl::SearchWorkspace& ws, uint64_t nq) {
  const uint32_t* status = ws.h_status;
  for (uint64_t i = 0; i < nq; i++) {
    if (status[i] == QS_OK) continue;
// ... 321 lines not shown
  const uint64_t d = idx->rows.d();
  {
    std::lock_guard<std::mutex> lock(idx->mu);
    if (isl::any_lane_busy(idx))
      return isl::fail(ISL_ERR_SEARCH, "Search error: isl_index_prepare while searches are in flight");
    ISL_TRY(isl::ensure_padded_adjacency(idx));
    ISL_TRY(ensure_pool(idx, idx->ws[0]));
    for (int i = 0; i < lanes; ++i) idx->ws[i].busy = true;
  }
  const uint32_t ovf_slots = (uint32_t)std::min<uint64_t>(max_nq, (uint64_t)isl::device_cu_count(idx->device) * kMaxWavesPerCu);
  CallGeometry cg_max;
  ISL_TRY(call_geometry(idx, d, max_k, max_ef, nullptr, cg_max));
  struct ReleaseAll {
    isl_index* idx; int lanes;
    ~ReleaseAll() { for (int i = 0; i < lanes; ++i) release_lane(idx, idx->ws[i]); }
  } release_all{idx, lanes};
  for (int i = 0; i < lanes; ++i) {
    isl::SearchWorkspace& ws = idx->ws[i];
    ISL_TRY(prepare_workspace(idx, ws, (uint32_t)max_nq, idx->recompute ? (uint32_t)max_nq : ovf_slots, cg_max.plog_cap));
    ISL_TRY(prepare_host_staging(ws, max_nq, d, std::max<uint64_t>(max_k, 1)));
    if (idx->recompute) ISL_TRY(prepare_recompute(ws, max_nq, cg_max.state_words));
    if (idx->is_hnsw) ISL_TRY(ws.q_entry.reserve(max_nq * 2, &ws.alloc_events));
    else if (idx->seeds.count()) ISL_TRY(ws.q_entry.reserve(max_nq * 4, &ws.alloc_events));
    if (idx->pq && idx->d_codes && !idx->is_hnsw && d == idx->pq->dimension)
      ISL_TRY(ws.tl_tables.reserve(max_nq * idx->pq->m * idx->pq->K, &ws.alloc_events));
    memset(ws.h_q, 0, max_nq * d * 4);
  }
  for (int round = 0; round < 2; ++round) {
    for (int i = 0; i < lanes; ++i) {
      isl::SearchWorkspace& ws = idx->ws[i];
      hipLaunchKernelGGL(copy_u128_kernel, dim3(256), dim3(256), 0, ws.stream, (const uint4*)ws.h_q.get(),
                         (uint4*)ws.q_stage.get(), max_nq * d * 4 / 16);
      const uint64_t efs[] = {max_ef, std::min<uint64_t>(max_ef, 64)};
      SearchCall warm_call;
      warm_call.d = d;
      for (uint64_t e : efs) {
        warm_call.k = std::min<uint64_t>(max_k, e);
        warm_call.ef = e;
        ISL_TRY(search_enqueue(idx, ws, warm_call, RoundPlan{}, true));
      }
      if (idx->pq && idx->d_codes && !idx->is_hnsw && d == idx->pq->dimension) {
        warm_call.k = std::min<uint64_t>(max_k, max_ef);
        warm_call.ef = max_ef;
        warm_call.two_level = true;
        warm_call.ratio = 0.5f;
        ISL_TRY(search_enqueue(idx, ws, warm_call, RoundPlan{}, true));
      }
      ws.publish_results = true;
      ISL_TRY(publish(ws, max_nq, std::max<uint64_t>(max_k, 1), ws.stream));
    }
    for (int i = 0; i < lanes; ++i) ISL_HIP(hipStreamSynchronize(idx->ws[i].stream));
  }
  for (int i = 0; i < lanes; ++i) idx->ws[i].alloc_mark = idx->ws[i].alloc_events;
  ISL_TRY(group_prepare(idx, max_nq, max_ef, max_k, lanes,
                        (uint32_t)(isl::device_cu_count(idx->device) * kMaxWavesPerCu), cg_max.plog_cap));
  return ISL_OK;
}

static isl_status search_batch_device(const isl_index* idx, const SearchCall& c) {
  isl::SearchWorkspace* ws = nullptr;
  bool answered = false;
  ISL_TRY(begin_call(idx, c, true, &ws, &answered));
  if (answered) return ISL_OK;
  LaneGuard guard{idx, ws};
  const isl_status st = search_sync(idx, *ws, c);
  note_last_stats(idx, ws->stats);
  return st;
}

static isl_status search_batch_device_async(const isl_index* idx, SearchCall c, uint64_t* token) {
  if (!token) return isl::fail(ISL_ERR_INVALID_ARGUMENT, "token is NULL");
  *token = 0;
  isl::SearchWorkspace* ws = nullptr;
  bool answered = false;
  ISL_TRY(begin_call(idx, c, true, &ws, &answered));
  if (answered) return ISL_OK;
  LaneGuard guard{idx, ws};
  if (idx->recompute || c.two_level) {
    ISL_TRY(order_after_user_stream(idx, *ws, c));
    ISL_TRY(start_worker(idx, ws, [=]() {
      return idx->recompute ? recompute_coalesced(idx, *ws, c) : search_sync(idx, *ws, c);
    }));
  } else if (group_takes(idx, c)) {
    ISL_TRY(group_arrive(idx, *ws, c));
  } else {
    c.mode = StreamMode::OWN_AFTER_USER;
    ISL_TRY(search_enqueue(idx, *ws, c));
  }
  issue_token(idx, *ws, token);
  guard.keep();
  return ISL_OK;
}

isl_status isl_search_batch_device(const isl_index* idx, const float* d_queries, uint64_t nq,
                                   uint64_t d, uint64_t k, uint64_t ef, uint64_t* d_out_ids,
                                   float* d_out_dist, uint32_t* d_out_count, void* stream) {
  return search_batch_device(idx, SearchCall{d_queries, nq, d, k, ef, d_out_ids, d_out_dist, d_out_count,
                                             (hipStream_t)stream, StreamMode::USER});
}

isl_status isl_search_batch_device_async(const isl_index* idx, const float* d_queries, uint64_t nq,
                                         uint64_t d, uint64_t k, uint64_t ef, uint64_t* d_out_ids,
                                         float* d_out_dist, uint32_t* d_out_count, void* stream,
                                         uint64_t* token) {
  return search_batch_device_async(idx, SearchCall{d_queries, nq, d, k, ef, d_out_ids, d_out_dist, d_out_count,
                                                   (hipStream_t)stream, StreamMode::USER}, token);
}

isl_status isl_search_batch_async(const isl_index* idx, const float* queries, uint64_t nq, uint64_t d,
                                  uint64_t k, uint64_t ef, uint64_t* out_ids, float* out_dist,
                                  uint32_t* out_count, uint64_t* token) {
  if (!token) return isl::fail(ISL_ERR_INVALID_ARGUMENT, "token is NULL");
  *token = 0;
  SearchCall c{queries, nq, d, k, ef, out_ids, out_dist, out_count};
  isl::SearchWorkspace* ws = nullptr;
  bool answered = false;
  ISL_TRY(begin_call(idx, c, false, &ws, &answered));
  if (answered) return ISL_OK;
  LaneGuard guard{idx, ws};
  ISL_TRY(host_stage_in(idx, *ws, c));
  if (idx->recompute) {
    ISL_HIP(hipEventRecord(ws->ev_in, ws->stream));
    ISL_TRY(start_worker(idx, ws, [=]() { return recompute_coalesced(idx, *ws, c); }));
  } else {
    ISL_TRY(search_enqueue(idx, *ws, c));
  }
  ws->u_ids = out_ids;
  ws->u_dist = out_dist;
  ws->u_count = out_count;
  issue_token(idx, *ws, token);
  guard.keep();
  return ISL_OK;
}

isl_status isl_search_wait_stats(const isl_index* idx, uint64_t token, isl_search_stats* stats) {
  if (!idx) return isl::fail(ISL_ERR_INVALID_ARGUMENT, "index is NULL");
  if (token == 0) {
    if (stats) *stats = isl_search_stats{};
    return ISL_OK;
  }
  ISL_TRY(isl::use_device(idx->device));
  isl::SearchWorkspace* ws = nullptr;
  {
    std::lock_guard<std::mutex> lock(idx->mu);
    for (auto& w : idx->ws)
      if (w.busy && w.token == token && !w.waiting) { ws = &w; w.waiting = true; break; }
  }
  if (!ws) return isl::fail(ISL_ERR_INVALID_ARGUMENT, "unknown or already completed search token");
  LaneGuard guard{idx, ws};
  isl_status st = ISL_OK;
  const bool grouped = ws->grp;
  if (grouped) {
    st = group_before_wait(idx, *ws);
    if (st == ISL_OK) st = search_finish(idx, *ws);
    group_after_wait(idx, *ws);
  } else {
    group_pump(idx);
    if (!join_worker(*ws, &st)) st = search_finish(idx, *ws);
  }
  if (st == ISL_OK && ws->u_count) host_copy_out(*ws, ws->nq_inflight, ws->k_inflight, ws->u_ids, ws->u_dist, ws->u_count);
  if (stats) *stats = ws->stats;
  note_last_stats(idx, ws->stats);
  return st;
}

isl_status isl_search_wait(const isl_index* idx, uint64_t token) { return isl_search_wait_stats(idx, token, nullptr); }

isl_status isl_search_stream_wait(const isl_index* idx, uint64_t token, void* stream) {
  if (!idx) return isl::fail(ISL_ERR_INVALID_ARGUMENT, "index is NULL");
  if (token == 0) return ISL_OK;
  ISL_TRY(isl::use_device(idx->device));
  isl::SearchWorkspace* found = nullptr;
  isl::SearchWorkspace* grouped = nullptr;
  {
    std::lock_guard<std::mutex> lock(idx->mu);
    for (auto& w : idx->ws)
      if (w.busy && w.token == token) {
        if (w.grp) { grouped = &w; break; }
        if (!w.threaded) {
          ISL_HIP(hipStreamWaitEvent((hipStream_t)stream, w.ev1, 0));
          return ISL_OK;
        }
        if (!w.worker) return ISL_OK;
        if (w.waiting) return isl::fail(ISL_ERR_INVALID_ARGUMENT, "the call is being waited for on another thread");
        found = &w;
        w.waiting = true;
        break;
      }
  }
  if (grouped) {
    if (group_before_wait(idx, *grouped) == ISL_OK) ISL_HIP(hipStreamWaitEvent((hipStream_t)stream, grouped->grp_ready, 0));
    return ISL_OK;
  }
  if (!found) return isl::fail(ISL_ERR_INVALID_ARGUMENT, "unknown or already completed search token");
  found->worker->join();
  delete found->worker;
  found->worker = nullptr;
  {
    std::lock_guard<std::mutex> lock(idx->mu);
    found->waiting = false;
  }
  return ISL_OK;
}

static isl_status search_batch_host(const isl_index* idx, SearchCall c) {
  uint64_t* const out_ids = c.ids;
  float* const out_dist = c.dist;
  uint32_t* const out_count = c.count;
  isl::SearchWorkspace* ws = nullptr;
  bool answered = false;
  ISL_TRY(begin_call(idx, c, false, &ws, &answered));
  if (answered) return ISL_OK;
  LaneGuard guard{idx, ws};
  ISL_TRY(host_stage_in(idx, *ws, c));
  const isl_status st = search_sync(idx, *ws, c);
  note_last_stats(idx, ws->stats);
  ISL_TRY(st);
  host_copy_out(*ws, c.nq, c.k, out_ids, out_dist, out_count);
  return ISL_OK;
}

isl_status isl_search_batch(const isl_index* idx, const float* queries, uint64_t nq, uint64_t d,
                            uint64_t k, uint64_t ef, uint64_t* out_ids, float* out_dist,
                            uint32_t* out_count) {
  return search_batch_host(idx, SearchCall{queries, nq, d, k, ef, out_ids, out_dist, out_count});
}

isl_status isl_index_set_pq_codes(isl_index* idx, const isl_pq* pq, const uint16_t* codes, uint64_t n,
                                  int32_t mem) {
  if (!idx || !pq || (!codes && n)) return isl::fail(ISL_ERR_INVALID_ARGUMENT, "NULL argument");
  if (n == 0) return isl::fail(ISL_ERR_EMPTY_COLLECTION, "Empty vector collection");
  if (idx->device < 0) return isl::fail(ISL_ERR_DEVICE, "call isl_index_upload before attaching PQ codes");
  if (pq->device != idx->device)
    return isl::fail(ISL_ERR_INVALID_ARGUMENT, "quantizer and index live on different devices");
  if (n > 0x7FFFFFFFull) return isl::fail(ISL_ERR_UNSUPPORTED, "more than 2^31 - 1 code rows");
  ISL_TRY(isl::use_device(idx->device));
  std::lock_guard<std::mutex> lock(idx->mu);
  if (isl::any_lane_busy(idx))
    return isl::fail(ISL_ERR_SEARCH, "Search error: PQ codes cannot be swapped while searches are in flight");
  idx->d_codes.reset();
  idx->pq = nullptr;
  idx->ncodes = 0;
  const size_t bytes = (size_t)n * pq->m * 2;
  isl::DeviceBuffer<uint16_t> d_codes;
  isl::DeviceBuffer<uint32_t> d_flag;
  ISL_TRY(d_codes.reserve(n * pq->m));
  ISL_HIP(hipMemcpy(d_codes, codes, bytes, mem == ISL_MEM_HOST ? hipMemcpyHostToDevice : hipMemcpyDeviceToDevice));
  ISL_TRY(d_flag.reserve(1));
  ISL_HIP(hipMemset(d_flag, 0, 4));
  hipLaunchKernelGGL(check_codes_kernel, dim3(1024), dim3(256), 0, nullptr, d_codes.get(), (uint64_t)n * pq->m,
                     (uint32_t)pq->K, d_flag.get());
  uint32_t flag = 0;
  hipError_t e = hipMemcpy(&flag, d_flag, 4, hipMemcpyDeviceToHost);
  if (e != hipSuccess) return isl::fail(ISL_ERR_DEVICE, "code check failed: %s", hipGetErrorString(e));
  if (flag) return isl::fail(ISL_ERR_PQ, "PQ error: a code is not below num_centroids = %llu", (unsigned long long)pq->K);
  idx->d_codes = std::move(d_codes);
  idx->pq = pq;
  idx->ncodes = n;
  return ISL_OK;
}

isl_status isl_search_two_level_batch(const isl_index* idx, const float* queries, uint64_t nq, uint64_t d,
                                      uint64_t k, uint64_t ef, float rerank_ratio, uint64_t* out_ids,
                                      float* out_dist, uint32_t* out_count) {
  return search_batch_host(idx, SearchCall{queries, nq, d, k, ef, out_ids, out_dist, out_count, nullptr,
                                           StreamMode::OWN, true, rerank_ratio});
}

isl_status isl_search_two_level_batch_device(const isl_index* idx, const float* d_queries, uint64_t nq,
                                             uint64_t d, uint64_t k, uint64_t ef, float rerank_ratio,
                                             uint64_t* d_out_ids, float* d_out_dist, uint32_t* d_out_count,
                                             void* stream) {
  return search_batch_device(idx, SearchCall{d_queries, nq, d, k, ef, d_out_ids, d_out_dist, d_out_count,
                                             (hipStream_t)stream, StreamMode::USER, true, rerank_ratio});
}

isl_status isl_search_two_level_batch_device_async(const isl_index* idx, const float* d_queries, uint64_t nq,
                                                   uint64_t d, uint64_t k, uint64_t ef, float rerank_ratio,
                                                   uint64_t* d_out_ids, float* d_out_dist, uint32_t* d_out_count,
                                                   void* stream, uint64_t* token) {
  return search_batch_device_async(idx, SearchCall{d_queries, nq, d, k, ef, d_out_ids, d_out_dist, d_out_count,
                                                   (hipStream_t)stream, StreamMode::USER, true, rerank_ratio}, token);
}

isl_status isl_search(const isl_index* idx, const float* query, uint64_t d, uint64_t k,
                      uint64_t* out_ids, float* out_dist, uint32_t* out_count) {
  if (!idx) return isl::fail(ISL_ERR_INVALID_ARGUMENT, "index is NULL");
  return isl_search_batch(idx, query, 1, d, k, idx->cfg.ef_search, out_ids, out_dist,
                          out_count);
}

isl_status isl_search_last_stats(const isl_index* idx, isl_search_stats* out) {
  if (!idx || !out) return isl::fail(ISL_ERR_INVALID_ARGUMENT, "NULL argument");
  *out = tl_last_stats.idx == idx ? tl_last_stats.st : isl_search_stats{};
  return ISL_OK;
}

}
```

### islands_amd/csrc/search_group.hip

```cpp
#include <memory>

#include "search_geometry.hpp"
#include "search_group_plan.hpp"
#include "search_internal.hpp"

using namespace isl_lane;

namespace isl {

struct GroupState {
  isl_group::Planner plan;
  std::vector<std::unique_ptr<SearchWorkspace>> slots;
  SearchCall calls[kSearchLanes];
  uint64_t launches = 0, shared_launches = 0, shared_calls = 0;
};

}

namespace {

struct GroupMember {
  const float* q;
  uint64_t* ids;
  float* dist;
  uint32_t* count;
  uint32_t* h_status;
  uint32_t* h_ctr;
  uint32_t* h_head;
  uint32_t offset, nq;
};
static_assert(sizeof(GroupMember) == 64, "member table rows are eight words");

constexpr uint32_t kMaxMembers = isl::kSearchLanes;
constexpr uint32_t kScatterBlocks = 64;

__global__ void group_gather_kernel(const GroupMember* __restrict__ tab, float* __restrict__ dst, uint32_t d) {
  const GroupMember m = tab[blockIdx.y];
  const uint64_t n = (uint64_t)m.nq * d;
  const float* __restrict__ src = m.q;
  float* __restrict__ out = dst + (uint64_t)m.offset * d;
  const uint64_t t = (uint64_t)blockIdx.x * blockDim.x + threadIdx.x;
  const uint64_t stride = (uint64_t)gridDim.x * blockDim.x;
  if (n % 4 == 0 && (((uintptr_t)src | (uintptr_t)out) & 15) == 0) {
    const uint4* __restrict__ s4 = reinterpret_cast<const uint4*>(src);
    uint4* __restrict__ o4 = reinterpret_cast<uint4*>(out);
    for (uint64_t i = t; i < n / 4; i += stride) o4[i] = s4[i];
  } else {
    for (uint64_t i = t; i < n; i += stride) out[i] = src[i];
  }
}

struct ScatterParams {
  const GroupMember* tab;
  const uint64_t* ids;
  const float* dist;
  const uint32_t* count;
  const uint32_t* status;
  const uint32_t* ctr;
  const uint32_t* redo;
  const uint2* plog;
  uint32_t* ticket;
  uint32_t* h_head;
  uint32_t* scratch;
  uint32_t k, ef, plog_cap;
};

__device__ __forceinline__ uint32_t wave_sum(uint32_t v) {
  for (int o = 32; o > 0; o >>= 1) v += (uint32_t)__shfl_xor((int)v, o);
  return v;
}

__global__ void group_scatter_kernel(ScatterParams sp) {
  const GroupMember m = sp.tab[blockIdx.y];
  const uint32_t lane = threadIdx.x & 63;
  const uint32_t wave = blockIdx.x * (blockDim.x >> 6) + (threadIdx.x >> 6);
  const uint32_t nwaves = gridDim.x * (blockDim.x >> 6);
  const uint32_t k = sp.k;
  const uint32_t nredo = *((volatile uint32_t*)&sp.ticket[1]);
  uint32_t n_exact = 0, n_replayed = 0;
  for (uint32_t qi = wave; qi < m.nq; qi += nwaves) {
    const uint32_t q = m.offset + qi;
    const uint32_t cnt = sp.count[q];
    const uint32_t st = sp.status[q];
    if (lane == 0) {
      m.count[qi] = cnt;
      m.h_status[qi] = st;
    }
    if (lane < 4) m.h_ctr[qi * 4 + lane] = sp.ctr[q * 4 + lane];
    const uint32_t outn = cnt < k ? cnt : k;
    for (uint32_t e = lane; e < outn; e += 64) {
      m.ids[(uint64_t)qi * k + e] = sp.ids[(uint64_t)q * k + e];
      m.dist[(uint64_t)qi * k + e] = sp.dist[(uint64_t)q * k + e];
    }
    bool hit = false;
    for (uint32_t i = lane; i < nredo; i += 64) hit |= sp.redo[i] == q;
    if (__ballot(hit)) { n_exact += 1; continue; }
    if (st != QS_OK || outn == 0) continue;
    const uint32_t* db = reinterpret_cast<const uint32_t*>(sp.dist) + (uint64_t)q * k;
    bool dup = false;
    for (uint32_t e = lane; e + 1 < outn; e += 64) dup |= db[e] == db[e + 1];
    bool tie = __ballot(dup) != 0;
    const uint32_t pushes = sp.ctr[q * 4 + 3];
    const uint32_t len = pushes < sp.ef ? pushes : sp.ef;
    if (!tie && outn == k && len >= k + 1) {
      const uint32_t dk = db[k - 1];
      uint32_t returned = 0, pushed = 0;
      for (uint32_t e = lane; e < k; e += 64) returned += db[e] == dk;
      const uint2* pl = sp.plog + (uint64_t)q * sp.plog_cap;
      const uint32_t logged = pushes < sp.plog_cap ? pushes : sp.plog_cap;
      for (uint32_t i = lane; i < logged; i += 64) pushed += pl[i].x == dk;
      tie = wave_sum(pushed) > wave_sum(returned);
    }
    if (tie && pushes <= sp.plog_cap) n_replayed += 1;
  }
  uint32_t* mine = sp.scratch + blockIdx.y * 4;
  if (lane == 0) {
    if (n_exact) atomicAdd(&mine[0], n_exact);
    if (n_replayed) atomicAdd(&mine[1], n_replayed);
  }
  __threadfence();
  __syncthreads();
  if (threadIdx.x != 0) return;
  if (atomicAdd(&mine[2], 1u) == gridDim.x - 1) {
    __threadfence();
    const uint32_t ex = atomicExch(&mine[0], 0u), rp = atomicExch(&mine[1], 0u);
    mine[2] = 0u;
    for (uint32_t i = 0; i < 16; ++i) m.h_head[i] = i == 1 ? ex : i == 3 ? rp : 0u;
  }
  uint32_t* all = sp.scratch + kMaxMembers * 4;
  if (atomicAdd(all, 1u) == gridDim.x * gridDim.y - 1) {
    *all = 0u;
    for (uint32_t i = 0; i < 16; ++i) {
      sp.h_head[i] = sp.ticket[i];
      sp.ticket[i] = 0u;
    }
  }
}

__global__ void zero_u32_kernel(uint32_t* p, uint32_t n) {
  for (uint32_t i = blockIdx.x * blockDim.x + threadIdx.x; i < n; i += gridDim.x * blockDim.x) p[i] = 0u;
}

uint32_t group_cap(const isl_index* idx) { return idx->group_sw.cap ? idx->group_sw.cap : isl_group::kDefaultCap; }

isl::GroupState& state_of(const isl_index* idx) {
  if (!idx->group) {
    idx->group = new isl::GroupState();
    idx->group->plan.configure(group_cap(idx), 0);
  }
  return *idx->group;
}

isl_status prepare_slot(const isl_index* idx, isl::SearchWorkspace& gw, uint64_t nq, uint64_t d, uint64_t k) {
  uint64_t* const ev = &gw.alloc_events;
  gw.union_launch = true;
  ISL_TRY(ensure_lane_stream(idx, gw));
  ISL_TRY(gw.q_stage.reserve(nq * d, ev));
  const uint64_t outs = nq * std::max<uint64_t>(k, 1);
  ISL_TRY(gw.ids_stage.reserve(outs, ev));
  ISL_TRY(gw.dist_stage.reserve(outs, ev));
  ISL_TRY(gw.count_stage.reserve(nq, ev));
  ISL_TRY(gw.h_members.reserve((uint64_t)kMaxMembers * 8, ev));
  if (!gw.grp_scratch) {
    ISL_TRY(gw.grp_scratch.reserve(kMaxMembers * 4 + 4, ev));
    hipLaunchKernelGGL(zero_u32_kernel, dim3(1), dim3(256), 0, gw.stream, gw.grp_scratch.get(), kMaxMembers * 4 + 4);
    ISL_HIP(hipGetLastError());
  }
  return ISL_OK;
}

isl::SearchWorkspace& slot(isl::GroupState& g, int32_t w) {
  if (!g.slots[w]) {
    g.slots[w].reset(new isl::SearchWorkspace());
    g.slots[w]->pool_lane = isl::kSearchLanes - 1 - w;
  }
  return *g.slots[w];
}

void grow_slots(const isl_index* idx, isl::GroupState& g, uint32_t n) {
  if (g.slots.size() < n) g.slots.resize(n);
  g.plan.configure(group_cap(idx), n);
}

isl_status enqueue_alone(const isl_index* idx, isl::GroupState& g, const isl_group::Launch& L) {
  const uint32_t lane_no = L.members[0].call;
  isl::SearchWorkspace& ws = idx->ws[lane_no];
  SearchCall c = g.calls[lane_no];
  c.user_stream = nullptr;
  c.mode = StreamMode::OWN_AFTER_EVENT;
  ISL_TRY(search_enqueue(idx, ws, c));
  ws.grp_launch = nullptr;
  ws.grp_offset = 0;
  ws.grp_ready = ws.ev1;
  return ISL_OK;
}

isl_status enqueue_group_impl(const isl_index* idx, isl::GroupState& g, const isl_group::Launch& L,
                              isl::SearchWorkspace& gw) {
  const uint64_t d = L.key.d, k = L.key.k;
  const uint32_t nm = (uint32_t)L.members.size();
  if (nm > kMaxMembers) return isl::fail(ISL_ERR_SEARCH, "Search error: %u calls in one group launch", nm);
  CallGeometry cg;
  ISL_TRY(call_geometry(idx, d, k, L.key.ef, nullptr, cg));
  ISL_TRY(prepare_slot(idx, gw, L.nq, d, k));
  ISL_TRY(prepare_workspace(idx, gw, L.nq, (uint32_t)std::min<uint64_t>(L.nq, cg.lane_slots), cg.plog_cap));
  GroupMember* tab = reinterpret_cast<GroupMember*>(gw.h_members.get());
  for (uint32_t i = 0; i < nm; ++i) {
    const isl_group::Member& mb = L.members[i];
    isl::SearchWorkspace& ws = idx->ws[mb.call];
    const SearchCall& c = g.calls[mb.call];
    ISL_TRY(ws.h_status.reserve(std::max<uint64_t>(mb.nq, 1024), &ws.alloc_events));
    ISL_TRY(ws.h_ctr.reserve(std::max<uint64_t>(mb.nq, 1024) * 4, &ws.alloc_events));
    tab[i] = GroupMember{c.queries, c.ids, c.dist, c.count, ws.h_status, ws.h_ctr, ws.h_head, mb.offset, mb.nq};
    ISL_HIP(hipStreamWaitEvent(gw.stream, ws.ev_in, 0));
  }
  hipLaunchKernelGGL(group_gather_kernel, dim3(64, nm), dim3(256), 0, gw.stream, tab, gw.q_stage.get(), (uint32_t)d);
  ISL_HIP(hipGetLastError());
  SearchCall u;
  u.queries = gw.q_stage;
  u.nq = L.nq;
  u.d = d;
  u.k = k;
  u.ef = L.key.ef;
  u.ids = gw.ids_stage;
  u.dist = gw.dist_stage;
  u.count = gw.count_stage;
  u.mode = StreamMode::OWN;
  ISL_TRY(search_enqueue(idx, gw, u));
  ScatterParams sp{};
  sp.tab = tab;
  sp.ids = gw.ids_stage;
  sp.dist = gw.dist_stage;
  sp.count = gw.count_stage;
  sp.status = gw.status;
  sp.ctr = gw.ctr;
  sp.redo = gw.redo;
  sp.plog = reinterpret_cast<const uint2*>(gw.plog.get());
  sp.ticket = gw.ticket;
  sp.h_head = gw.h_head;
  sp.scratch = gw.grp_scratch;
  sp.k = (uint32_t)k;
  sp.ef = cg.ef;
  sp.plog_cap = cg.plog_cap;
  hipLaunchKernelGGL(group_scatter_kernel, dim3(kScatterBlocks, nm), dim3(256), 0, gw.stream, sp);
  ISL_HIP(hipGetLastError());
  gw.ticket_clean = true;
  ISL_HIP(hipEventRecord(gw.ev_done, gw.stream));
  return ISL_OK;
}

isl_status enqueue_group(const isl_index* idx, isl::GroupState& g, const isl_group::Launch& L) {
  isl::SearchWorkspace& gw = slot(g, L.workspace);
  const uint64_t mark = gw.alloc_events;
  const isl_status st = enqueue_group_impl(idx, g, L, gw);
  gw.enqueued = false;
  if (st != ISL_OK) {
    const isl::ErrorRecord keep = isl::last_error();
    if (gw.stream) (void)hipStreamSynchronize(gw.stream);
    (void)hipGetLastError();
    gw.ticket_clean = false;
    isl::last_error() = keep;
    return st;
  }
  for (const isl_group::Member& mb : L.members) {
    isl::SearchWorkspace& ws = idx->ws[mb.call];
    ws.grp_launch = &gw;
    ws.grp_offset = mb.offset;
    ws.grp_ready = gw.ev_done;
    ws.grp_allocs = gw.alloc_events - mark;
    ws.enqueued = true;
    ws.nq_inflight = mb.nq;
    ws.k_inflight = L.key.k;
    ws.ef_inflight = gw.ef_inflight;
    ws.fast_inflight = gw.fast_inflight;
    ws.st_inflight = gw.stream;
  }
  return ISL_OK;
}

void poll(const isl_index* idx, isl::GroupState& g) {
  for (const isl_group::Planner::Live& l : g.plan.live()) {
    hipEvent_t ev = l.workspace >= 0 ? g.slots[l.workspace]->ev_done : idx->ws[l.first_call].ev_done;
    const hipError_t e = hipEventQuery(ev);
    if (e == hipSuccess) g.plan.complete(l.id);
    else (void)hipGetLastError();
  }
}

void submit(const isl_index* idx, isl::GroupState& g, uint32_t wanted) {
  isl_group::Launch L;
  for (;;) {
    if (wanted != isl_group::kNone && !g.plan.held(wanted)) wanted = isl_group::kNone;
    if (!g.plan.next(wanted, L)) break;
    const isl_status st = L.workspace < 0 ? enqueue_alone(idx, g, L) : enqueue_group(idx, g, L);
    if (st == ISL_OK) {
      g.launches += 1;
      if (L.workspace >= 0) { g.shared_launches += 1; g.shared_calls += L.members.size(); }
      continue;
    }
    for (const isl_group::Member& mb : L.members) {
      isl::SearchWorkspace& ws = idx->ws[mb.call];
      ws.grp_failed = true;
      ws.grp_status = st;
      ws.grp_error = isl::last_error();
      ws.grp_launch = nullptr;
      ws.enqueued = false;
    }
    g.plan.abandon(L.id);
  }
}

}

bool isl_lane::group_takes(const isl_index* idx, const SearchCall& c) {
  static const bool instrumented = getenv("ISL_TIMELINE") != nullptr || getenv("ISL_DEBUG") != nullptr;
  isl_group::CallTraits t;
  t.device_async = true;
  t.recompute = idx->recompute;
  t.two_level = c.two_level;
  t.hnsw = idx->is_hnsw;
  t.construction = idx->build_q_entry != nullptr;
  t.instrumented = instrumented;
  t.nq = c.nq;
  return isl_group::groupable(t, idx->group_sw.off, group_cap(idx));
}

isl_status isl_lane::group_arrive(const isl_index* idx, isl::SearchWorkspace& ws, const SearchCall& c) {
  CallGeometry cg;
  ISL_TRY(call_geometry(idx, c.d, c.k, c.ef, nullptr, cg));
  ISL_TRY(ensure_lane_stream(idx, ws));
  ISL_HIP(hipEventRecord(ws.ev_in, c.user_stream));
  const uint32_t lane_no = (uint32_t)(&ws - idx->ws);
  std::lock_guard<std::mutex> lock(idx->group_mu);
  isl::GroupState& g = state_of(idx);
  if (g.slots.empty()) grow_slots(idx, g, isl::kSearchLanes / 2);
  g.calls[lane_no] = c;
  ws.grp = true;
  ws.grp_failed = false;
  ws.grp_launch = nullptr;
  ws.grp_allocs = 0;
  poll(idx, g);
  const uint32_t room = idx->group_sw.room ? idx->group_sw.room : cg.slots;
  g.plan.arrive(lane_no, (uint32_t)c.nq, isl_group::Key{c.d, c.k, cg.ef}, room);
  submit(idx, g, isl_group::kNone);
  if (ws.grp_failed) {
    ws.grp = false;
    isl::last_error() = ws.grp_error;
    return ws.grp_status;
  }
  return ISL_OK;
}

void isl_lane::group_pump(const isl_index* idx) {
  std::lock_guard<std::mutex> lock(idx->group_mu);
  if (!idx->group || !idx->group->plan.any_held()) return;
  poll(idx, *idx->group);
  submit(idx, *idx->group, isl_group::kNone);
}

isl_status isl_lane::group_before_wait(const isl_index* idx, isl::SearchWorkspace& ws) {
  std::lock_guard<std::mutex> lock(idx->group_mu);
  isl::GroupState& g = state_of(idx);
  poll(idx, g);
  submit(idx, g, (uint32_t)(&ws - idx->ws));
  if (ws.grp_failed) {
    isl::last_error() = ws.grp_error;
    return ws.grp_status;
  }
  return ISL_OK;
}

void isl_lane::group_after_wait(const isl_index* idx, isl::SearchWorkspace& ws) {
  std::lock_guard<std::mutex> lock(idx->group_mu);
  if (!idx->group) return;
  isl::GroupState& g = *idx->group;
  const isl::ErrorRecord keep = isl::last_error();
  g.plan.finished((uint32_t)(&ws - idx->ws));
  ws.grp = false;
  ws.grp_launch = nullptr;
  if (g.plan.any_held()) {
    poll(idx, g);
    submit(idx, g, isl_group::kNone);
  }
  isl::last_error() = keep;
}

isl_status isl_lane::group_prepare(const isl_index* idx, uint64_t max_nq, uint64_t max_ef, uint64_t max_k, int32_t lanes,
                                   uint32_t ovf_waves, uint32_t plog_cap) {
  if (idx->group_sw.off || idx->recompute || idx->is_hnsw || idx->build_q_entry) return ISL_OK;
  std::lock_guard<std::mutex> lock(idx->group_mu);
  isl::GroupState& g = state_of(idx);
  const uint32_t cap = group_cap(idx);
  const uint32_t n = isl_group::workspaces_for((uint32_t)lanes, max_nq, cap);
  const uint64_t nq = isl_group::workspace_queries((uint32_t)lanes, max_nq, cap);
  grow_slots(idx, g, std::max<uint32_t>(n, (uint32_t)g.slots.size()));
  const uint64_t d = idx->rows.d();
  for (uint32_t w = 0; w < n; ++w) {
    isl::SearchWorkspace& gw = slot(g, (int32_t)w);
    ISL_TRY(prepare_slot(idx, gw, nq, d, std::max<uint64_t>(max_k, 1)));
    ISL_TRY(prepare_workspace(idx, gw, (uint32_t)nq, (uint32_t)std::min<uint64_t>(nq, ovf_waves), plog_cap));
    if (idx->seeds.count()) ISL_TRY(gw.q_entry.reserve(nq * 4, &gw.alloc_events));
  }
  for (int round = 0; round < 2; ++round) {
    for (uint32_t w = 0; w < n; ++w) {
      isl::SearchWorkspace& gw = *g.slots[w];
      GroupMember* tab = reinterpret_cast<GroupMember*>(gw.h_members.get());
      tab[0] = GroupMember{};
      hipLaunchKernelGGL(group_gather_kernel, dim3(1, 1), dim3(256), 0, gw.stream, tab, gw.q_stage.get(), (uint32_t)d);
      ISL_HIP(hipGetLastError());
      SearchCall warm_call;
      warm_call.d = d;
      warm_call.k = std::min<uint64_t>(max_k, max_ef);
      warm_call.ef = max_ef;
      ISL_TRY(search_enqueue(idx, gw, warm_call, RoundPlan{}, true));
      ScatterParams sp{};
      sp.tab = tab;
      sp.ids = gw.ids_stage;
      sp.dist = gw.dist_stage;
      sp.count = gw.count_stage;
      sp.status = gw.status;
      sp.ctr = gw.ctr;
      sp.redo = gw.redo;
      sp.plog = reinterpret_cast<const uint2*>(gw.plog.get());
      sp.ticket = gw.ticket;
      sp.h_head = gw.h_head;
      sp.scratch = gw.grp_scratch;
      sp.k = (uint32_t)std::max<uint64_t>(max_k, 1);
      sp.ef = (uint32_t)max_ef;
      sp.plog_cap = plog_cap;
      tab[0].h_head = gw.h_head;
      hipLaunchKernelGGL(group_scatter_kernel, dim3(kScatterBlocks, 1), dim3(256), 0, gw.stream, sp);
      ISL_HIP(hipGetLastError());
      gw.ticket_clean = true;
      ISL_HIP(hipEventRecord(gw.ev_done, gw.stream));
    }
    for (uint32_t w = 0; w < n; ++w) ISL_HIP(hipStreamSynchronize(g.slots[w]->stream));
  }
  return ISL_OK;
}

extern "C" isl_status isl_index_group_counters(const isl_index* idx, uint64_t* launches, uint64_t* shared_launches,
                                               uint64_t* shared_calls) {
  if (!idx) return isl::fail(ISL_ERR_INVALID_ARGUMENT, "index is NULL");
  std::lock_guard<std::mutex> lock(idx->group_mu);
  const isl::GroupState* g = idx->group;
  if (launches) *launches = g ? g->launches : 0;
  if (shared_launches) *shared_launches = g ? g->shared_launches : 0;
  if (shared_calls) *shared_calls = g ? g->shared_calls : 0;
  return ISL_OK;
}

void isl::free_group_state(isl_index* idx) {
// ... 15 lines not shown
```

### islands_amd/csrc/search_internal.hpp

```cpp
#pragma once

#include "common.hpp"

namespace isl_lane __attribute__((visibility("hidden"))) {

enum class StreamMode { OWN, USER, OWN_AFTER_USER, OWN_AFTER_EVENT };

struct SearchCall {
  const float* queries = nullptr;
  uint64_t nq = 0, d = 0, k = 0, ef = 0;
  uint64_t* ids = nullptr;
  float* dist = nullptr;
  uint32_t* count = nullptr;
  hipStream_t user_stream = nullptr;
  StreamMode mode = StreamMode::OWN;
  bool two_level = false;
  float ratio = 0.0f;
};
inline hipStream_t call_stream(const isl::SearchWorkspace& ws, const SearchCall& c) {
  return c.mode == StreamMode::USER ? c.user_stream : ws.stream;
}

struct RoundPlan {
  uint32_t active = 0;
  uint32_t exact = 0;
  bool exact_parks = false;
  bool listed = false;
  uint32_t prefetch = 0;
  uint32_t retry = 0;
  uint32_t window_scale = 1;
  bool tables_built = false;
};

isl_status ensure_lane_stream(const isl_index* idx, isl::SearchWorkspace& ws);
isl_status ensure_pool(const isl_index* idx, isl::SearchWorkspace& ws);
void copy_words(const uint32_t* src, uint32_t* dst, uint64_t n, uint32_t grid, uint32_t block, hipStream_t st);
isl_status prepare_workspace(const isl_index* idx, isl::SearchWorkspace& ws, uint32_t nq, uint32_t slots,
                             uint32_t plog_cap);
isl_status search_enqueue(const isl_index* idx, isl::SearchWorkspace& ws, const SearchCall& c,
                          const RoundPlan& plan = RoundPlan{}, bool warm = false);
isl_status search_finish(const isl_index* idx, isl::SearchWorkspace& ws, uint32_t* misses = nullptr,
                         bool defer_statuses = false);
isl_status search_statuses(isl::SearchWorkspace& ws, uint64_t nq);
isl_status search_sync(const isl_index* idx, isl::SearchWorkspace& ws, const SearchCall& c);

isl_status prepare_recompute(isl::SearchWorkspace& ws, uint64_t nq, uint64_t state_words_per_query);
isl_status tl_retry_short(isl::SearchWorkspace& ws, uint64_t nq, uint32_t& window_scale, uint32_t* nshort);
isl_status recompute_rounds(const isl_index* idx, isl::SearchWorkspace& ws, const SearchCall& c);
isl_status recompute_coalesced(const isl_index* idx, isl::SearchWorkspace& ws, const SearchCall& c);

bool group_takes(const isl_index* idx, const SearchCall& c);
isl_status group_arrive(const isl_index* idx, isl::SearchWorkspace& ws, const SearchCall& c);
void group_pump(const isl_index* idx);
isl_status group_before_wait(const isl_index* idx, isl::SearchWorkspace& ws);
void group_after_wait(const isl_index* idx, isl::SearchWorkspace& ws);
isl_status group_prepare(const isl_index* idx, uint64_t max_nq, uint64_t max_ef, uint64_t max_k, int32_t lanes,
                         uint32_t ovf_waves, uint32_t plog_cap);

}
```

### islands_amd/csrc/search_kernels.hip.h

```cpp
#pragma once
#include "device_common.hip.h"
#include "encoder.hpp"
#include "query_status.hpp"

#include <algorithm>
#include <type_traits>

namespace {

using namespace isl_dev;

constexpr uint32_t EMPTY = 0xFFFFFFFFu;
constexpr uint32_t FLAG_EXP = 0x80000000u;
constexpr uint32_t ID_MASK = 0x7FFFFFFFu;


struct SearchParams {
  const uint64_t* off;
  const uint32_t* adj;
  uint64_t num_nodes;
  const void* emb;
  uint32_t emb_bf16;
  const float* norm2;
  uint64_t nvec;
  uint64_t stride;
  uint32_t d;
  const float* queries;
  uint32_t nq;
  uint32_t k, ef;
  float prune_ratio;
  uint32_t prune_strategy;
  uint32_t entry;
  uint64_t* out_ids;
  float* out_dist;
  uint32_t* out_count;
  uint32_t* status;
  uint64_t* payload;
  uint32_t* ctr;
  uint32_t* ticket;
  uint32_t* redo;
  uint32_t* replay;
  uint64_t* prof;
  uint64_t* tline;
  uint2* plog;
  uint32_t plog_cap;
  uint32_t hbits;
  uint32_t hcap;
  uint32_t* otab;
  uint32_t obits;
  float* cand_d;
  uint32_t* cand_id;
  uint64_t cand_cap;
  uint32_t* vis_bits;
  uint64_t vis_words;
  uint32_t* ulist;
  uint32_t ulist_cap;
  uint32_t* pool_locks;
  uint32_t pool_slots;
  uint32_t* xslot;
  uint32_t* xstate;
  uint32_t xstate_words;
  uint32_t ell_w;
  const uint32_t* ell_deg;
  const uint32_t* slot_of;
  uint32_t* stamp;
  uint32_t round_no;
  uint32_t* miss;
  uint32_t miss_cap;
  uint32_t* qstate;
  uint32_t qstate_words;
  uint32_t* qflag;
  const uint32_t* qlist;
  uint32_t* qsel;
  uint32_t* qsel_h;
  uint32_t qsel_mode;
  const uint64_t* const* layer_off;
  const uint32_t* const* layer_adj;
  uint32_t max_level;
  uint32_t hnsw_order;
  uint32_t seq_max;
  uint32_t* q_entry;
  uint32_t* q_evals;
  uint32_t entry_given;
  const float* tl_tables;
  const uint16_t* tl_codes;
  uint64_t tl_ncodes;
  uint32_t tl_m, tl_K;
  float tl_ratio;
  uint32_t tl_wcap;
  uint32_t tl_prefetch;
  uint32_t* pref;
  uint32_t pref_cap;
};

constexpr uint32_t KEY_MAX = 0xFFFFFFFFu;

__device__ __forceinline__ float key_to_dist(uint32_t k) {
  return __uint_as_float((k & 0x80000000u) ? (k & 0x7FFFFFFFu) : ~k);
}

__device__ __forceinline__ bool odd_distance(float d) {
  return d != d || __float_as_uint(d) == 0x80000000u;
}

template <int S>
struct RSet {
  uint32_t kd[S];
  uint32_t id[S];
  uint32_t len;

  __device__ __forceinline__ void init() {
#pragma unroll
    for (int s = 0; s < S; ++s) { kd[s] = KEY_MAX; id[s] = KEY_MAX; }
    len = 0;
  }
  __device__ __forceinline__ uint32_t key_at(uint32_t e) const {
    uint32_t r = 0;
#pragma unroll
    for (int s = 0; s < S; ++s)
      if ((int)(e >> 6) == s) r = rl_u(kd[s], e & 63);
    return r;
  }
  __device__ __forceinline__ uint32_t id_at(uint32_t e) const {
    uint32_t r = 0;
#pragma unroll
    for (int s = 0; s < S; ++s)
      if ((int)(e >> 6) == s) r = rl_u(id[s], e & 63);
    return r;
  }
  __device__ __forceinline__ uint32_t first_unexpanded() const {
#pragma unroll
    for (int s = 0; s < S; ++s) {
      uint64_t m = ballot(!(id[s] & FLAG_EXP));
      if (m) return s * 64 + (uint32_t)__ffsll((long long)m) - 1;
    }
    return 0xFFFFFFFFu;
  }
  __device__ __forceinline__ void mark_expanded(uint32_t e) {
    const int lane = threadIdx.x;
#pragma unroll
    for (int s = 0; s < S; ++s)
      if ((int)(e >> 6) == s && lane == (int)(e & 63)) id[s] |= FLAG_EXP;
  }
  __device__ __forceinline__ void insert(uint32_t nk, uint32_t nid, uint32_t cap) {
    const uint32_t lane = threadIdx.x;
    uint32_t pos = 0;
#pragma unroll
    for (int s = 0; s < S; ++s) {
      const uint64_t lt = ballot(kd[s] < nk);
      const uint64_t eq = ballot(kd[s] == nk);
      const uint64_t il = ballot((id[s] & ID_MASK) < nid);
      pos += (uint32_t)__popcll(lt | (eq & il));
    }
#pragma unroll
    for (int s = S - 1; s >= 0; --s) {
      if (pos >= 64u * (uint32_t)(s + 1)) continue;
      uint32_t uk = shr1_u(kd[s]);
      uint32_t ui = shr1_u(id[s]);
      if (s > 0) {
        const uint32_t pk = rl_u(kd[s - 1], 63), pi = rl_u(id[s - 1], 63);
        uk = lane == 0 ? pk : uk;
        ui = lane == 0 ? pi : ui;
      }
      const uint32_t e = (uint32_t)s * 64u + lane;
      const bool mv = e > pos && e < cap;
      kd[s] = mv ? uk : kd[s];
      id[s] = mv ? ui : id[s];
      const bool here = e == pos;
      kd[s] = here ? nk : kd[s];
      id[s] = here ? nid : id[s];
    }
  }
};

constexpr uint32_t kBatchMax = 32;
__host__ __device__ constexpr uint32_t mbuf_entries(uint32_t ef) { return ef + kBatchMax > 64u ? ef + kBatchMax : 64u; }
constexpr int BI_DONE = 1, BI_FALLBACK = 0, BI_TIE = 2;
// ... 259 lines not shown
  const uint64_t am = ballot(absent);
  if (!am) return true;
  uint32_t base = 0;
  if (lane == 0) base = atomicAdd(&p.ticket[13], (uint32_t)__popcll(am));
  base = uni(base);
  const uint32_t rank = (uint32_t)__popcll(am & ((1ull << lane) - 1ull));
  if (absent && base + rank < p.miss_cap) p.miss[base + rank] = uid;
  return false;
}
__device__ __forceinline__ bool rows_present2(const SearchParams& p, uint32_t uid_lo, uint32_t n_lo,
                                              uint32_t uid_hi, uint32_t n_hi) {
  if (!p.slot_of) return true;
  const uint32_t lane = threadIdx.x;
  const uint32_t s_lo = lane < n_lo ? p.slot_of[uid_lo] : 0u, s_hi = lane < n_hi ? p.slot_of[uid_hi] : 0u;
  const bool a_lo = lane < n_lo && s_lo >= kSlotClaim;
  const bool a_hi = lane < n_hi && s_hi >= kSlotClaim;
  if (lane < n_lo && !a_lo) p.stamp[s_lo] = p.round_no;
  if (lane < n_hi && !a_hi) p.stamp[s_hi] = p.round_no;
  const uint64_t m_lo = ballot(a_lo), m_hi = ballot(a_hi);
  if (!(m_lo | m_hi)) return true;
  const uint32_t c_lo = (uint32_t)__popcll(m_lo);
  uint32_t base = 0;
  if (lane == 0) base = atomicAdd(&p.ticket[13], c_lo + (uint32_t)__popcll(m_hi));
  base = uni(base);
  const uint64_t below = (1ull << lane) - 1ull;
  if (a_lo && base + (uint32_t)__popcll(m_lo & below) < p.miss_cap) p.miss[base + (uint32_t)__popcll(m_lo & below)] = uid_lo;
  if (a_hi && base + c_lo + (uint32_t)__popcll(m_hi & below) < p.miss_cap)
    p.miss[base + c_lo + (uint32_t)__popcll(m_hi & below)] = uid_hi;
  return false;
}
__device__ __forceinline__ uint32_t row_index(const SearchParams& p, uint32_t id, bool live) {
  if (!p.slot_of) return id;
  return live ? p.slot_of[id] : 0u;
}

__device__ __forceinline__ bool visited_insert(uint32_t* htab, uint32_t hcap, bool ovf,
                                               uint32_t* otab, uint32_t obits, uint32_t omask, uint32_t id,
                                               bool act) {
  bool fresh = false;
  if (act) {
    uint32_t h = hslot_cap(id, hcap);
    if (!ovf) {
      for (;;) {
        uint32_t old = atomicCAS(&htab[h], EMPTY, id);
        if (old == EMPTY) { fresh = true; break; }
        if (old == id) break;
        h = h + 1 == hcap ? 0u : h + 1;
      }
    } else {
      bool found = false;
      for (;;) {
        uint32_t cur = htab[h];
        if (cur == id) { found = true; break; }
        if (cur == EMPTY) break;
        h = h + 1 == hcap ? 0u : h + 1;
      }
      if (!found) {
        uint32_t g = hslot(id, obits);
        for (;;) {
          uint32_t old = atomicCAS(&otab[g], EMPTY, id);
          if (old == EMPTY) { fresh = true; break; }
          if (old == id) break;
          g = (g + 1) & omask;
        }
      }
    }
  }
  return fresh;
}

__global__ __launch_bounds__(64) void classify_queries_kernel(SearchParams p) {
  const uint32_t lane = threadIdx.x;
  for (uint32_t qi = blockIdx.x; qi < p.nq; qi += gridDim.x) {
    const uint32_t* q = reinterpret_cast<const uint32_t*>(p.queries + (uint64_t)qi * p.d);
    bool bad = false;
    for (uint32_t j = lane; j < p.d; j += 64) bad |= (q[j] & 0xFFFFu) != 0u;
    if (lane == 0) {
      if (ballot(bad)) p.qsel[atomicAdd(&p.ticket[5], 1u)] = qi;
      else p.qsel_h[atomicAdd(&p.ticket[7], 1u)] = qi;
    }
  }
}

template <int S, int METRIC_API, typename ROWT, bool WIDE, bool RESUME = false, bool QH = false>
__global__ __launch_bounds__(64) __attribute__((amdgpu_waves_per_eu(3))) void leann_search_fast(SearchParams p) {
  static_assert(!QH || (sizeof(ROWT) == 2 && !RESUME), "the bf16 query operand goes with bf16 rows");
  constexpr uint32_t kMaxDeg = WIDE ? 128u : 64u;
  constexpr uint32_t kStTie = 16, kStHop = 80, kStR = 208, kStTab = 208 + S * 128;
  constexpr int METRIC = METRIC_API == ISL_METRIC_COSINE ? METRIC_COSINE_PRE : METRIC_API;
  const ROWT* const emb = reinterpret_cast<const ROWT*>(p.emb);
  extern __shared__ __align__(16) unsigned char smem[];
  const int lane = threadIdx.x;
  const uint32_t hcap = p.hcap;
  const uint32_t hlimit = hcap - hcap / 8;
  uint32_t* htab = reinterpret_cast<uint32_t*>(smem);
  uint32_t* mbuf = htab + hcap;
  uint32_t* scratch = mbuf;
  float* qs = reinterpret_cast<float*>(mbuf + 2 * mbuf_entries(p.ef));
  const uint32_t ocap = 1u << p.obits;
  const uint32_t omask = ocap - 1;
  const uint32_t olimit = ocap - ocap / 4;
  uint32_t* otab = p.otab + (size_t)blockIdx.x * ocap;
  const uint32_t ef = p.ef;

  for (;;) {
    uint32_t qi = 0;
    if constexpr (sizeof(ROWT) == 2 && !QH && !RESUME) {
      if (p.qsel_mode) {
        if (lane == 0) qi = atomicAdd(&p.ticket[6], 1u);
        qi = uni(qi);
        if (qi >= *((volatile uint32_t*)&p.ticket[5])) break;
        qi = p.qsel[qi];
      } else {
        if (lane == 0) qi = atomicAdd(&p.ticket[0], 1u);
        qi = uni(qi);
        if (qi >= p.nq) break;
      }
    } else if constexpr (QH) {
      if (lane == 0) qi = atomicAdd(&p.ticket[4], 1u);
      qi = uni(qi);
      if (qi >= *((volatile uint32_t*)&p.ticket[7])) break;
      qi = p.qsel_h[qi];
    } else {
      if (lane == 0) qi = atomicAdd(&p.ticket[0], 1u);
      qi = uni(qi);
      if (qi >= p.nq) break;
    }
    if constexpr (RESUME) {
      if (p.qlist) qi = p.qlist[qi];
      otab = p.otab + (size_t)qi * ocap;
    }

    if (p.q_entry && p.status[qi] != QS_OK) {
      if (lane == 0) {
        p.out_count[qi] = 0;
        p.ctr[qi * 4 + 0] = 0; p.ctr[qi * 4 + 1] = 0; p.ctr[qi * 4 + 2] = p.q_evals[qi]; p.ctr[qi * 4 + 3] = 0;
      }
      continue;
    }
    const uint64_t t_start = __builtin_amdgcn_s_memrealtime();
    bool resumed = false;
    uint32_t* qst = nullptr;
    if constexpr (RESUME) {
      qst = p.qstate + (size_t)qi * p.qstate_words;
      resumed = uni(p.qflag[qi]) == 1u;
    }
    if (resumed) { for (uint32_t i = lane; i < hcap; i += 64) htab[i] = qst[kStTab + i]; }
    else { for (uint32_t i = lane; i < hcap; i += 64) htab[i] = EMPTY; }
    float q_norm;
    if constexpr (QH) {
      bool representable;
      q_norm = load_query_bf16<METRIC>(p.queries + (uint64_t)qi * p.d, p.d, qs, &representable);
      if (!representable) {
        if (lane == 0) p.qsel[atomicAdd(&p.ticket[5], 1u)] = qi;
        continue;
      }
    } else {
      q_norm = load_query<METRIC>(p.queries + (uint64_t)qi * p.d, p.d, qs);
    }

    RSet<S> rs;
    rs.init();
    uint32_t hcount = 0, ocount = 0;
    bool ovf = false;
    uint32_t status = QS_OK;
    uint64_t payload = 0;
// ... 236 lines not shown
          rs.insert(id_k, id_i, ef);
          rs.len += 1;
        }
        cP += 1;
        pending &= ~((2ull << r) - 1ull);
        if (r == 63) pending = 0;
      }
      ISL_MARK(tp3)
     } while (WIDE && (sbase += 64) < keep_all && status == QS_OK);
    }

    uint32_t outn = rs.len < p.k ? rs.len : p.k;
    if (status == QS_OK) {
      uint32_t chk = rs.len < p.k + 1 ? rs.len : p.k + 1;
      bool tie = false;
#pragma unroll
      for (int s = 0; s < S; ++s) {
        uint32_t e = s * 64 + lane;
        uint32_t nxt = (uint32_t)__shfl_down((int)rs.kd[s], 1);
        if (s + 1 < S) {
          uint32_t nd0 = rl_u(rs.kd[s + 1 < S ? s + 1 : s], 0);
          if (lane == 63) nxt = nd0;
        }
        if (e + 1 < chk && rs.kd[s] == nxt) tie = true;
      }
      if (ballot(tie)) {
        if (cP <= p.plog_cap) status = QS_REPLAY;
        else { status = QS_REDO; payload = 4; }
      }
    }
    if (status == QS_REPLAY) {
      __threadfence_block();
      __syncthreads();
      float* res_d = reinterpret_cast<float*>(htab);
      uint32_t* res_i = htab + (ef + 1);
      uint2* stage = reinterpret_cast<uint2*>(htab + 2 * (ef + 1));
      replay_result_order(plog, cP, ef, p.k, qi, res_d, res_i, stage, p.out_ids, p.out_dist,
                          p.out_count);
      status = QS_OK;
      outn = 0xFFFFFFFFu;
      if (lane == 0) atomicAdd(&p.ticket[3], 1u);
    }
    if (status == QS_OK && outn != 0xFFFFFFFFu) {
#pragma unroll
      for (int s = 0; s < S; ++s) {
        uint32_t e = s * 64 + lane;
        if (e < outn) {
          p.out_ids[(uint64_t)qi * p.k + e] = (uint64_t)(rs.id[s] & ID_MASK);
          p.out_dist[(uint64_t)qi * p.k + e] = key_to_dist(rs.kd[s]);
        }
      }
    }
    if (lane == 0) {
      p.status[qi] = status;
      p.payload[qi] = status == QS_OK ? (__builtin_amdgcn_s_memrealtime() - t_start) : payload;
      if (outn != 0xFFFFFFFFu) p.out_count[qi] = status == QS_OK ? outn : 0u;
      p.ctr[qi * 4 + 0] = cH;
      p.ctr[qi * 4 + 1] = cE;
      p.ctr[qi * 4 + 2] = cV;
      p.ctr[qi * 4 + 3] = cP;
      if (p.tline) {
        p.tline[qi * 2] = t_start;
        p.tline[qi * 2 + 1] = ((__builtin_amdgcn_s_memrealtime() - t_start) & 0xFFFFFFFFFFull) | ((uint64_t)cH << 40);
      }
      if (p.prof) {
        p.prof[qi * 8 + 0] = tp0; p.prof[qi * 8 + 1] = tp1; p.prof[qi * 8 + 2] = tp2; p.prof[qi * 8 + 3] = tp3;
        p.prof[qi * 8 + 4] = ngroups; p.prof[qi * 8 + 5] = nhops_rows;
      }
      if (status == QS_REDO) {
        p.redo[atomicAdd(&p.ticket[1], 1u)] = qi;
        atomicAdd(&p.ticket[payload == 5 ? 12u : payload == 6 ? 14u : 8u + ((uint32_t)payload & 3u)], 1u);
      }
    }
    bool parked = false;
    if constexpr (RESUME) {
      parked = status == QS_BLOCKED && have_hop;
      if (!parked && lane == 0) p.qflag[qi] = 0u;
    }
    if (ovf && !parked) {
      for (uint32_t i = lane; i < ocap; i += 64) otab[i] = EMPTY;
    }
    wave_sync();
  }
}


template <int METRIC>
__device__ __forceinline__ float exact_rows(const SearchParams& p, uint32_t rid, uint32_t R,
                                            const float* qs, float* tile, float q_norm, float aux) {
  if (p.emb_bf16)
    return lane_distances_bf16<METRIC>(reinterpret_cast<const uint16_t*>(p.emb), p.stride, p.d, rid, R, qs,
                                       q_norm, aux);
  return wave_distances<METRIC>(reinterpret_cast<const float*>(p.emb), p.stride, p.d, rid, R, qs, tile, q_norm, aux);
}

template <int METRIC_API, bool HNSW>
__global__ __launch_bounds__(64) void leann_search_exact(SearchParams p) {
  constexpr int METRIC = METRIC_API == ISL_METRIC_COSINE ? METRIC_COSINE_PRE : METRIC_API;
  using CandOrd = typename std::conditional<HNSW, HnswCandOrder, CandOrder>::type;
  using ResOrd = typename std::conditional<HNSW, HnswResultOrder, ResultOrder>::type;
  extern __shared__ __align__(16) unsigned char smem[];
  const int lane = threadIdx.x;
  const uint32_t ef = p.ef;
  float* tile = reinterpret_cast<float*>(smem);
  uint32_t* scratch = reinterpret_cast<uint32_t*>(tile + TILE_ROWS * TILE_LD);
  float* dscratch = reinterpret_cast<float*>(scratch + 64);
  uint32_t* ctl = reinterpret_cast<uint32_t*>(dscratch + 64);
  float* res_d = reinterpret_cast<float*>(ctl + 8);
  uint32_t* res_i = reinterpret_cast<uint32_t*>(res_d + (ef + 1));
  float* qs = reinterpret_cast<float*>(res_i + (ef + 1));
  qs = reinterpret_cast<float*>(((uintptr_t)qs + 15) & ~(uintptr_t)15);

  uint32_t slot = 0xFFFFFFFFu;
  float* cand_d = nullptr;
  uint32_t* cand_i = nullptr;
  uint32_t* vis = nullptr;
  uint32_t* ulist = nullptr;

  for (;;) {
    uint32_t t = 0;
    if (lane == 0) t = atomicAdd(&p.ticket[2], 1u);
    t = uni(t);
    uint32_t nredo = *((volatile uint32_t*)&p.ticket[1]);
    if (t >= nredo) break;
    const uint32_t qi = p.redo[t];
    bool xresumed = false;
    if (p.xslot) {
      const uint32_t xs = uni(p.xslot[qi]);
      uint32_t sl = 0xFFFFFFFFu;
      if (xs) {
        sl = xs - 1u;
        xresumed = true;
      } else if (slot != 0xFFFFFFFFu) {
        sl = slot;
      } else {
        if (lane == 0) {
          for (uint32_t tries = 0; tries < 2u * p.pool_slots && sl == 0xFFFFFFFFu; ++tries) {
            const uint32_t c = (blockIdx.x + tries) % p.pool_slots;
            if (atomicCAS(&p.pool_locks[c], 0u, 1u) == 0u) sl = c;
          }
        }
        sl = uni(sl);
        if (sl == 0xFFFFFFFFu) {
          if (lane == 0) {
            p.status[qi] = QS_BLOCKED;
            p.out_count[qi] = 0;
            p.ctr[qi * 4 + 0] = 0; p.ctr[qi * 4 + 1] = 0; p.ctr[qi * 4 + 2] = 0; p.ctr[qi * 4 + 3] = 0;
          }
          continue;
        }
      }
      if (sl != slot) {
        if (slot != 0xFFFFFFFFu && lane == 0) atomicExch(&p.pool_locks[slot], 0u);
        slot = sl;
        __builtin_amdgcn_fence(__ATOMIC_ACQUIRE, "agent");
        cand_d = p.cand_d + (size_t)slot * p.cand_cap;
        cand_i = p.cand_id + (size_t)slot * p.cand_cap;
        vis = p.vis_bits + (size_t)slot * p.vis_words;
        ulist = p.ulist + (size_t)slot * p.ulist_cap;
      }
    } else
    if (slot == 0xFFFFFFFFu) {
      uint32_t sl = 0;
      if (lane == 0) {
        sl = blockIdx.x % p.pool_slots;
        while (atomicCAS(&p.pool_locks[sl], 0u, 1u) != 0u) {
// ... 695 lines not shown
```

Before: 1.602 million queries/s.

## Add lean launch sequence that folds publish into fast kernel and defers exact pass

For async entry points, the fast search kernel's last workgroup now copies statuses, counters and ticket head straight into pinned host memory and resets the ticket, replacing the separate publish step. The exact fallback kernel is no longer launched unconditionally; it is enqueued at wait time only when redo entries exist. The input event record is skipped when the caller's stream is idle. This removes several launches, memsets and event operations per batch, at the cost of extra host-side follow-up logic, and the exact pass can only start once the host waits.

```diff
diff --git a/include/islands_amd.h b/include/islands_amd.h
--- a/include/islands_amd.h
+++ b/include/islands_amd.h
@@ -182,6 +182,8 @@
 isl_status isl_search_stream_wait(const isl_index* idx, uint64_t token, void* stream);
 isl_status isl_index_group_counters(const isl_index* idx, uint64_t* launches, uint64_t* shared_launches,
                                     uint64_t* shared_calls);
+isl_status isl_index_launch_counters(const isl_index* idx, uint64_t* lean_calls, uint64_t* late_exact,
+                                     uint64_t* stream_wait_exact, uint64_t* events_elided);
 isl_status isl_search(const isl_index* idx, const float* query, uint64_t d, uint64_t k,
                       uint64_t* out_ids, float* out_dist, uint32_t* out_count);
 
diff --git a/include/islands_amd.hpp b/include/islands_amd.hpp
--- a/include/islands_amd.hpp
+++ b/include/islands_amd.hpp
@@ -223,6 +223,12 @@
   }
   void prepare(uint64_t max_nq, uint64_t max_ef, uint64_t max_k = 10, int32_t lanes = 8) {
     check(isl_index_prepare(h_, max_nq, max_ef, max_k, lanes));
+  }
+  struct LaunchCounters { uint64_t lean_calls = 0, late_exact = 0, stream_wait_exact = 0, events_elided = 0; };
+  LaunchCounters launch_counters() const {
+    LaunchCounters c;
+    check(isl_index_launch_counters(h_, &c.lean_calls, &c.late_exact, &c.stream_wait_exact, &c.events_elided));
+    return c;
   }
   std::vector<std::pair<uint64_t, float>> search(const std::vector<float>& query, uint64_t k) const {
     return search_with_params(query, k, config().ef_search);
diff --git a/islands_amd/__init__.py b/islands_amd/__init__.py
--- a/islands_amd/__init__.py
+++ b/islands_amd/__init__.py
@@ -724,6 +724,11 @@
         s = SearchStatsC()
         _check(_ffi.lib().isl_search_last_stats(self._h, C.byref(s)))
         return {f: getattr(s, f) for f, _ in SearchStatsC._fields_}
+
+    def launch_counters(self) -> dict:
+        v = [C.c_uint64() for _ in range(4)]
+        _check(_ffi.lib().isl_index_launch_counters(self._h, *[C.byref(x) for x in v]))
+        return dict(zip(("lean_calls", "late_exact", "stream_wait_exact", "events_elided"), (int(x.value) for x in v)))
 
 
 def merge_topk(ids, scores, counts, top_k: int, id_base=None, device: int = 0):
diff --git a/islands_amd/_ffi.py b/islands_amd/_ffi.py
--- a/islands_amd/_ffi.py
+++ b/islands_amd/_ffi.py
@@ -102,6 +102,7 @@
     "isl_search_wait": (i32, [C.c_void_p, u64]),
     "isl_search_stream_wait": (i32, [C.c_void_p, u64, C.c_void_p]),
     "isl_index_group_counters": (i32, [C.c_void_p, P(u64), P(u64), P(u64)]),
+    "isl_index_launch_counters": (i32, [C.c_void_p, P(u64), P(u64), P(u64), P(u64)]),
     "isl_shard_record_bytes": (u64, [u64, u64]),
     "isl_merge_topk_packed_async": (i32, [u64, u64, u64, C.c_void_p, u64, C.c_void_p, u64, C.c_void_p, C.c_void_p,
                                           C.c_void_p, C.c_void_p, C.c_void_p, i32, C.c_void_p]),
diff --git a/islands_amd/csrc/common.hpp b/islands_amd/csrc/common.hpp
--- a/islands_amd/csrc/common.hpp
+++ b/islands_amd/csrc/common.hpp
@@ -97,6 +97,7 @@
   PinnedBuffer<uint32_t> h_status;
   PinnedBuffer<uint32_t> h_ctr;
   PinnedBuffer<uint32_t> h_head;
+  PinnedBuffer<uint64_t> h_lean;
   DeviceBuffer<uint64_t> d_prof;
   DeviceBuffer<uint64_t> d_tline;
   DeviceBuffer<uint32_t> q_entry;
@@ -124,6 +125,14 @@
   uint64_t alloc_events = 0;
   uint64_t alloc_mark = 0;
   isl_search_stats stats{};
+  bool ev_in_recorded = false;
+  bool lean = false;
+  bool lean_exact = false;
+  const float* lean_queries = nullptr;
+  uint64_t lean_d = 0;
+  uint64_t* lean_ids = nullptr;
+  float* lean_dist = nullptr;
+  uint32_t* lean_count = nullptr;
   bool grp = false;
   SearchWorkspace* grp_launch = nullptr;
   uint32_t grp_offset = 0;
@@ -136,6 +145,7 @@
   bool union_launch = false;
   PinnedBuffer<uint64_t> h_members;
   DeviceBuffer<uint32_t> grp_scratch;
+  uint32_t grp_members = 0, grp_plog_cap = 0;
 };
 
 constexpr int kSearchLanes = 32;
@@ -154,6 +164,10 @@
   return GroupSwitches{is_off, num("ISL_GROUP_CAP"), num("ISL_GROUP_ROOM")};
 }
 struct GroupState;
+inline bool lean_launch_off() {
+  const char* e = getenv("ISL_LEAN_LAUNCH");
+  return e && strcmp(e, "0") == 0;
+}
 
 struct ExactPool {
   uint32_t slots = 0;
@@ -247,6 +261,8 @@
   const isl::GroupSwitches group_sw = isl::group_switches();
   mutable std::mutex group_mu;
   mutable isl::GroupState* group = nullptr;
+  const bool lean_off = isl::lean_launch_off();
+  mutable std::atomic<uint64_t> lean_calls{0}, late_exact{0}, stream_wait_exact{0}, events_elided{0};
 };
 
 struct isl_hnsw {
diff --git a/islands_amd/csrc/lean_launch_plan.hpp b/islands_amd/csrc/lean_launch_plan.hpp
--- /dev/null
+++ b/islands_amd/csrc/lean_launch_plan.hpp
@@ -0,0 +1,50 @@
+#pragma once
+
+#include <cstdint>
+
+namespace isl_lean {
+
+enum class Entry : uint8_t {
+  DEVICE_SYNC,
+  HOST_SYNC,
+  DEVICE_ASYNC,
+  GROUP_MEMBER,
+  HOST_ASYNC,
+  WARM,
+};
+
+struct CallTraits {
+  Entry entry = Entry::DEVICE_SYNC;
+  bool recompute = false;
+  bool two_level = false;
+  bool hnsw = false;
+  bool construction = false;
+  bool use_fast = false;
+};
+
+enum class Sequence : uint8_t { CLASSIC, LEAN };
+inline Sequence sequence(const CallTraits& t, bool lean_off) {
+  const bool lean_entry = t.entry == Entry::DEVICE_ASYNC || t.entry == Entry::GROUP_MEMBER || t.entry == Entry::HOST_ASYNC;
+  return !lean_off && lean_entry && !t.recompute && !t.two_level && !t.hnsw && !t.construction && t.use_fast
+             ? Sequence::LEAN : Sequence::CLASSIC;
+}
+
+enum class Wait : uint8_t { HOST, STREAM };
+enum class Followup : uint8_t {
+  NONE,
+  EXACT_NOW,
+  EXACT_BEHIND,
+};
+struct FlightState {
+  Sequence seq = Sequence::CLASSIC;
+  bool exact_enqueued = false;
+  bool complete = false;
+  uint32_t redo = 0;
+};
+inline Followup followup(const FlightState& f, Wait w) {
+  if (f.seq == Sequence::CLASSIC || f.exact_enqueued) return Followup::NONE;
+  if (w == Wait::HOST || f.complete) return f.redo ? Followup::EXACT_NOW : Followup::NONE;
+  return Followup::EXACT_BEHIND;
+}
+
+}
diff --git a/islands_amd/csrc/search.hip b/islands_amd/csrc/search.hip
--- a/islands_amd/csrc/search.hip
+++ b/islands_amd/csrc/search.hip
@@ -82,8 +82,22 @@
     ws.ticket_clean = false;
   }
   ISL_TRY(ws.h_head.reserve(16, &ws.alloc_events));
+  ISL_TRY(ws.h_lean.reserve(8, &ws.alloc_events));
   ws.stream = st;
   return ISL_OK;
+}
+
+bool isl_lane::caller_stream_busy(hipStream_t user_stream) {
+  if (user_stream) {
+    hipStreamCaptureStatus cap = hipStreamCaptureStatusNone;
+    if (hipStreamIsCapturing(user_stream, &cap) != hipSuccess || cap != hipStreamCaptureStatusNone) {
+      (void)hipGetLastError();
+      return true;
+    }
+  }
+  if (hipStreamQuery(user_stream) == hipSuccess) return false;
+  (void)hipGetLastError();
+  return true;
 }
 
 void isl_lane::copy_words(const uint32_t* src, uint32_t* dst, uint64_t n, uint32_t grid, uint32_t block, hipStream_t st) {
@@ -212,6 +226,18 @@
   }
 }
 
+isl_lean::CallTraits lean_traits(const isl_index* idx, const SearchCall& c, const CallGeometry& cg, bool warm) {
+  isl_lean::CallTraits lt;
+  lt.entry = warm ? isl_lean::Entry::WARM : c.entry;
+  lt.recompute = idx->recompute;
+  lt.two_level = c.two_level;
+  lt.hnsw = idx->is_hnsw;
+  lt.construction = idx->build_q_entry != nullptr;
+  lt.use_fast = cg.use_fast && lean_kernel((int)cg.segments, (int)idx->cfg.metric, idx->rows.is_bf16(),
+                                                       idx->max_degree > 64, false, false);
+  return lt;
+}
+
 isl_status search_enqueue_impl(const isl_index* idx, isl::SearchWorkspace& ws, const SearchCall& c,
                                const RoundPlan& plan, bool warm) {
   const uint64_t nq = c.nq, d = c.d, k = c.k;
@@ -225,7 +251,10 @@
   const bool resume = !warm && (plan.active != 0 || plan.exact != 0);
   const bool tl_qh = tl && !warm && !resume && idx->rows.is_bf16() && plan.retry == 0 && cg.tl_hbits_q == cg.fg.hbits;
   const bool qh = cg.qh && !resume;
-  if (!warm)
+  const bool exact_pass = plan.exact_pass;
+  const isl_lean::CallTraits lt = lean_traits(idx, c, cg, warm);
+  const bool lean = !exact_pass && isl_lean::sequence(lt, idx->lean_off) == isl_lean::Sequence::LEAN;
+  if (!warm && !plan.exact_pass)
     ISL_TRY(prepare_workspace(idx, ws, (uint32_t)nq,
                               (uint32_t)(idx->recompute ? nq : std::min<uint64_t>(nq, cg.lane_slots)), cg.plog_cap));
   if (!idx->pool.slots || ((use_fast || (tl && idx->max_degree <= 128)) && !idx->d_ell && idx->d_off && idx->num_nodes)) {
@@ -236,10 +265,13 @@
     if (idx->d_ell != before) ws.alloc_events += 2;
   }
   hipStream_t st = call_stream(ws, c);
-  if (c.mode == StreamMode::OWN_AFTER_USER || c.mode == StreamMode::OWN_AFTER_EVENT) {
-    if (c.mode == StreamMode::OWN_AFTER_USER) ISL_HIP(hipEventRecord(ws.ev_in, c.user_stream));
+  if (c.mode == StreamMode::OWN_AFTER_USER) {
+    ws.ev_in_recorded = caller_stream_busy(c.user_stream);
+    if (ws.ev_in_recorded) ISL_HIP(hipEventRecord(ws.ev_in, c.user_stream));
+    else idx->events_elided.fetch_add(1, std::memory_order_relaxed);
+  }
+  if ((c.mode == StreamMode::OWN_AFTER_USER || c.mode == StreamMode::OWN_AFTER_EVENT) && ws.ev_in_recorded)
     ISL_HIP(hipStreamWaitEvent(ws.stream, ws.ev_in, 0));
-  }
 
   SearchParams p{};
   p.off = idx->d_off;
@@ -268,21 +300,20 @@
   p.ctr = ws.ctr;
   p.ticket = ws.ticket;
   p.redo = ws.redo;
-  ws.d_prof.reset();
+  if (!exact_pass) ws.d_prof.reset();
   static const bool debug_env = getenv("ISL_DEBUG") != nullptr;
-  if (debug_env && !warm) {
+  if (debug_env && !warm && !exact_pass) {
     ISL_TRY(ws.d_prof.reserve(nq * 8));
     ISL_HIP(hipMemset(ws.d_prof, 0, nq * 64));
   }
   p.prof = ws.d_prof;
   static const char* tline_env = getenv("ISL_TIMELINE");
-  ws.d_tline.reset();
-  if (tline_env && !warm) {
+  if (!exact_pass) ws.d_tline.reset();
+  if (tline_env && !warm && !exact_pass) {
     ISL_TRY(ws.d_tline.reserve(nq * 2));
     ISL_HIP(hipMemset(ws.d_tline, 0, nq * 16));
   }
   p.tline = ws.d_tline;
-  p.replay = ws.replay;
   p.plog = reinterpret_cast<uint2*>(ws.plog.get());
   p.plog_cap = cg.plog_cap;
   p.hbits = cg.fg.hbits;
@@ -356,9 +387,11 @@
   const uint64_t nq_grid = warm ? 1 : nq;
   const int metric = (int)idx->cfg.metric;
 
-  if (!ws.ticket_clean) ISL_HIP(hipMemsetAsync(ws.ticket, 0, 64, st));
-  ws.ticket_clean = false;
-  ISL_HIP(hipEventRecord(ws.ev0, st));
+  if (!exact_pass) {
+    if (!ws.ticket_clean) ISL_HIP(hipMemsetAsync(ws.ticket, 0, 64, st));
+    ws.ticket_clean = false;
+    ISL_HIP(hipEventRecord(ws.ev0, st));
+  }
   if (resume && !tl && plan.exact) {
     hipLaunchKernelGGL(seed_redo_kernel, dim3(1), dim3(256), 0, st, ws.h_xlist, plan.exact, ws.redo, ws.ticket);
     ISL_HIP(hipGetLastError());
@@ -393,7 +426,7 @@
     isl_launch::launch_descent(metric, dgrid, cg.descent_lds, st, &p);
     ISL_HIP(hipGetLastError());
   }
-  if (seeded) {
+  if (seeded && !exact_pass) {
     ISL_TRY(isl::launch_entry_pick(idx, c.queries, nq, ws.q_entry, ws.q_entry + nq,
                                    reinterpret_cast<unsigned long long*>(ws.q_entry + 2 * nq), ws.status, nullptr, st));
   }
@@ -403,7 +436,15 @@
     uint32_t grid = (uint32_t)std::min<uint64_t>(resume ? plan.active : nq_grid, cg.slots);
     const bool skip_fast = resume && plan.active == 0;
     isl_launch::FastKernel fk{cg.segments, metric, idx->max_degree > 64, p.emb_bf16 != 0, resume, false};
-    if (qh) {
+    if (lean) {
+      uint64_t* t = ws.h_lean;
+      t[0] = ws.union_launch ? 0 : (uint64_t)(uintptr_t)ws.h_status.get();
+      t[1] = ws.union_launch ? 0 : (uint64_t)(uintptr_t)ws.h_ctr.get();
+      t[2] = (uint64_t)(uintptr_t)ws.h_head.get();
+      p.lean_grid = grid;
+    }
+    if (exact_pass) {
+    } else if (qh) {
       p.qsel = ws.qsel;
       p.qsel_h = ws.qsel_h;
       isl_launch::launch_classify((uint32_t)std::min<uint64_t>(nq_grid, 2048), st, &p);
@@ -417,12 +458,15 @@
       p.hcap = cg.fg.hcap;
       p.qsel_mode = 1;
       fk.qh = false;
+      if (lean) p.lean = ws.h_lean;
       launch_fast(fk, grid, cg.fg.lds, st, p);
       p.qsel_mode = 0;
     } else if (!skip_fast) {
+      if (lean) p.lean = ws.h_lean;
       launch_fast(fk, grid, cg.fg.lds, st, p);
     }
     ISL_HIP(hipGetLastError());
+    p.lean = nullptr;
     p.nq = (uint32_t)nq;
   } else if (!warm && !resume) {
     std::vector<uint32_t> all(nq);
@@ -432,19 +476,30 @@
     ISL_HIP(hipMemcpyAsync(ws.ticket, head0, 16, hipMemcpyHostToDevice, st));
     ISL_HIP(hipStreamSynchronize(st));
   }
-  if (!tl) {
+  if (!tl && !lean) {
     uint32_t grid = (uint32_t)std::min<uint64_t>(nq_grid, idx->pool.slots);
     isl_launch::launch_exact(metric, idx->is_hnsw, grid, cg.exact_lds, st, &p);
     ISL_HIP(hipGetLastError());
   }
-  ISL_HIP(hipEventRecord(ws.ev1, st));
+  if (!exact_pass) ISL_HIP(hipEventRecord(ws.ev1, st));
   ws.st_inflight = st;
   if (warm) return ISL_OK;
 
   if (!ws.union_launch) {
-    ISL_TRY(publish(ws, nq, k, st));
+    if (!lean) ISL_TRY(publish(ws, nq, k, st));
     ISL_HIP(hipEventRecord(ws.ev_done, st));
   }
+  if (lean) {
+    ws.ticket_clean = true;
+    ws.lean_queries = c.queries;
+    ws.lean_d = d;
+    ws.lean_ids = c.ids;
+    ws.lean_dist = c.dist;
+    ws.lean_count = c.count;
+    if (!ws.union_launch) idx->lean_calls.fetch_add(1, std::memory_order_relaxed);
+  }
+  ws.lean = lean || exact_pass;
+  ws.lean_exact = exact_pass;
   ws.enqueued = true;
   ws.nq_inflight = nq;
   ws.k_inflight = k;
@@ -477,6 +532,40 @@
   return st;
 }
 
+isl_status isl_lane::lean_followup(const isl_index* idx, isl::SearchWorkspace& ws, isl_lean::Wait wait, bool* added) {
+  *added = false;
+  isl_lean::FlightState f;
+  f.seq = ws.lean ? isl_lean::Sequence::LEAN : isl_lean::Sequence::CLASSIC;
+  f.exact_enqueued = ws.lean_exact;
+  if (ws.lean && !ws.lean_exact) {
+    f.complete = wait == isl_lean::Wait::HOST;
+    if (!f.complete) {
+      f.complete = hipEventQuery(ws.ev_done) == hipSuccess;
+      if (!f.complete) (void)hipGetLastError();
+    }
+    if (f.complete) f.redo = ws.h_head[1];
+  }
+  if (isl_lean::followup(f, wait) == isl_lean::Followup::NONE) return ISL_OK;
+  SearchCall c;
+  c.queries = ws.lean_queries;
+  c.nq = ws.nq_inflight;
+  c.d = ws.lean_d;
+  c.k = ws.k_inflight;
+  c.ef = ws.ef_inflight;
+  c.ids = ws.lean_ids;
+  c.dist = ws.lean_dist;
+  c.count = ws.lean_count;
+  RoundPlan plan;
+  plan.exact_pass = true;
+  const bool enqueued = ws.enqueued;
+  const isl_status st = search_enqueue(idx, ws, c, plan);
+  ws.enqueued = enqueued;
+  ISL_TRY(st);
+  (wait == isl_lean::Wait::HOST ? idx->late_exact : idx->stream_wait_exact).fetch_add(1, std::memory_order_relaxed);
+  *added = true;
+  return ISL_OK;
+}
+
 isl_status isl_lane::search_finish(const isl_index* idx, isl::SearchWorkspace& ws, uint32_t* misses,
                                      bool defer_statuses) {
   if (!ws.enqueued) return isl::fail(ISL_ERR_INVALID_ARGUMENT, "no search in flight for this token");
@@ -485,6 +574,10 @@
   const bool use_fast = ws.fast_inflight;
   const isl::SearchWorkspace& lw = ws.grp_launch ? *ws.grp_launch : ws;
   ISL_HIP(hipEventSynchronize(lw.ev_done));
+  bool again = false;
+  if (ws.grp_launch) ISL_TRY(group_late_exact(idx, ws, &again));
+  else ISL_TRY(lean_followup(idx, ws, isl_lean::Wait::HOST, &again));
+  if (again) ISL_HIP(hipEventSynchronize(lw.ev_done));
   const uint32_t* status = ws.h_status;
   const uint32_t* ctr = ws.h_ctr;
   const uint32_t* head = ws.h_head;
@@ -972,8 +1065,10 @@
       return idx->recompute ? recompute_coalesced(idx, *ws, c) : search_sync(idx, *ws, c);
     }));
   } else if (group_takes(idx, c)) {
+    c.entry = isl_lean::Entry::DEVICE_ASYNC;
     ISL_TRY(group_arrive(idx, *ws, c));
   } else {
+    c.entry = isl_lean::Entry::DEVICE_ASYNC;
     c.mode = StreamMode::OWN_AFTER_USER;
     ISL_TRY(search_enqueue(idx, *ws, c));
   }
@@ -1013,6 +1108,16 @@
     ISL_HIP(hipEventRecord(ws->ev_in, ws->stream));
     ISL_TRY(start_worker(idx, ws, [=]() { return recompute_coalesced(idx, *ws, c); }));
   } else {
+    c.entry = isl_lean::Entry::HOST_ASYNC;
+    CallGeometry cg;
+    ISL_TRY(call_geometry(idx, d, k, ef, nullptr, cg));
+    const isl_lean::CallTraits lt = lean_traits(idx, c, cg, false);
+    if (isl_lean::sequence(lt, idx->lean_off) == isl_lean::Sequence::LEAN) {
+      c.ids = ws->h_ids;
+      c.dist = ws->h_dist;
+      c.count = ws->h_count;
+      ws->publish_results = false;
+    }
     ISL_TRY(search_enqueue(idx, *ws, c));
   }
   ws->u_ids = out_ids;
@@ -1062,15 +1167,13 @@
   ISL_TRY(isl::use_device(idx->device));
   isl::SearchWorkspace* found = nullptr;
   isl::SearchWorkspace* grouped = nullptr;
+  isl::SearchWorkspace* plain = nullptr;
   {
     std::lock_guard<std::mutex> lock(idx->mu);
     for (auto& w : idx->ws)
       if (w.busy && w.token == token) {
         if (w.grp) { grouped = &w; break; }
-        if (!w.threaded) {
-          ISL_HIP(hipStreamWaitEvent((hipStream_t)stream, w.ev1, 0));
-          return ISL_OK;
-        }
+        if (!w.threaded) { plain = &w; break; }
         if (!w.worker) return ISL_OK;
         if (w.waiting) return isl::fail(ISL_ERR_INVALID_ARGUMENT, "the call is being waited for on another thread");
         found = &w;
@@ -1078,8 +1181,17 @@
         break;
       }
   }
+  if (plain) {
+    bool added = false;
+    ISL_TRY(lean_followup(idx, *plain, isl_lean::Wait::STREAM, &added));
+    ISL_HIP(hipStreamWaitEvent((hipStream_t)stream, plain->lean ? plain->ev_done : plain->ev1, 0));
+    return ISL_OK;
+  }
   if (grouped) {
-    if (group_before_wait(idx, *grouped) == ISL_OK) ISL_HIP(hipStreamWaitEvent((hipStream_t)stream, grouped->grp_ready, 0));
+    if (group_before_wait(idx, *grouped) == ISL_OK) {
+      ISL_TRY(group_stream_ready(idx, *grouped));
+      ISL_HIP(hipStreamWaitEvent((hipStream_t)stream, grouped->grp_ready, 0));
+    }
     return ISL_OK;
   }
   if (!found) return isl::fail(ISL_ERR_INVALID_ARGUMENT, "unknown or already completed search token");
@@ -1180,6 +1292,16 @@
                           out_count);
 }
 
+isl_status isl_index_launch_counters(const isl_index* idx, uint64_t* lean_calls, uint64_t* late_exact,
+                                     uint64_t* stream_wait_exact, uint64_t* events_elided) {
+  if (!idx) return isl::fail(ISL_ERR_INVALID_ARGUMENT, "index is NULL");
+  if (lean_calls) *lean_calls = idx->lean_calls.load(std::memory_order_relaxed);
+  if (late_exact) *late_exact = idx->late_exact.load(std::memory_order_relaxed);
+  if (stream_wait_exact) *stream_wait_exact = idx->stream_wait_exact.load(std::memory_order_relaxed);
+  if (events_elided) *events_elided = idx->events_elided.load(std::memory_order_relaxed);
+  return ISL_OK;
+}
+
 isl_status isl_search_last_stats(const isl_index* idx, isl_search_stats* out) {
   if (!idx || !out) return isl::fail(ISL_ERR_INVALID_ARGUMENT, "NULL argument");
   *out = tl_last_stats.idx == idx ? tl_last_stats.st : isl_search_stats{};
diff --git a/islands_amd/csrc/search_group.hip b/islands_amd/csrc/search_group.hip
--- a/islands_amd/csrc/search_group.hip
+++ b/islands_amd/csrc/search_group.hip
@@ -63,6 +63,7 @@
   uint32_t* h_head;
   uint32_t* scratch;
   uint32_t k, ef, plog_cap;
+  uint32_t lean;
 };
 
 __device__ __forceinline__ uint32_t wave_sum(uint32_t v) {
@@ -130,7 +131,7 @@
   uint32_t* all = sp.scratch + kMaxMembers * 4;
   if (atomicAdd(all, 1u) == gridDim.x * gridDim.y - 1) {
     *all = 0u;
-    for (uint32_t i = 0; i < 16; ++i) {
+    for (uint32_t i = 0; i < 16 && !sp.lean; ++i) {
       sp.h_head[i] = sp.ticket[i];
       sp.ticket[i] = 0u;
     }
@@ -182,6 +183,38 @@
   g.plan.configure(group_cap(idx), n);
 }
 
+isl_status scatter(isl::SearchWorkspace& gw, bool lean) {
+  ScatterParams sp{};
+  sp.tab = reinterpret_cast<const GroupMember*>(gw.h_members.get());
+  sp.ids = gw.ids_stage;
+  sp.dist = gw.dist_stage;
+  sp.count = gw.count_stage;
+  sp.status = gw.status;
+  sp.ctr = gw.ctr;
+  sp.redo = gw.redo;
+  sp.plog = reinterpret_cast<const uint2*>(gw.plog.get());
+  sp.ticket = gw.ticket;
+  sp.h_head = gw.h_head;
+  sp.scratch = gw.grp_scratch;
+  sp.k = (uint32_t)gw.k_inflight;
+  sp.ef = gw.ef_inflight;
+  sp.plog_cap = gw.grp_plog_cap;
+  sp.lean = lean ? 1u : 0u;
+  hipLaunchKernelGGL(group_scatter_kernel, dim3(kScatterBlocks, gw.grp_members), dim3(256), 0, gw.stream, sp);
+  ISL_HIP(hipGetLastError());
+  gw.ticket_clean = true;
+  ISL_HIP(hipEventRecord(gw.ev_done, gw.stream));
+  return ISL_OK;
+}
+
+isl_status group_followup(const isl_index* idx, isl::SearchWorkspace& gw, isl_lean::Wait wait) {
+  bool added = false;
+  ISL_TRY(lean_followup(idx, gw, wait, &added));
+  gw.enqueued = false;
+  if (added) ISL_TRY(scatter(gw, false));
+  return ISL_OK;
+}
+
 isl_status enqueue_alone(const isl_index* idx, isl::GroupState& g, const isl_group::Launch& L) {
   const uint32_t lane_no = L.members[0].call;
   isl::SearchWorkspace& ws = idx->ws[lane_no];
@@ -191,7 +224,7 @@
   ISL_TRY(search_enqueue(idx, ws, c));
   ws.grp_launch = nullptr;
   ws.grp_offset = 0;
-  ws.grp_ready = ws.ev1;
+  ws.grp_ready = ws.lean ? ws.ev_done : ws.ev1;
   return ISL_OK;
 }
 
@@ -212,7 +245,7 @@
     ISL_TRY(ws.h_status.reserve(std::max<uint64_t>(mb.nq, 1024), &ws.alloc_events));
     ISL_TRY(ws.h_ctr.reserve(std::max<uint64_t>(mb.nq, 1024) * 4, &ws.alloc_events));
     tab[i] = GroupMember{c.queries, c.ids, c.dist, c.count, ws.h_status, ws.h_ctr, ws.h_head, mb.offset, mb.nq};
-    ISL_HIP(hipStreamWaitEvent(gw.stream, ws.ev_in, 0));
+    if (ws.ev_in_recorded) ISL_HIP(hipStreamWaitEvent(gw.stream, ws.ev_in, 0));
   }
   hipLaunchKernelGGL(group_gather_kernel, dim3(64, nm), dim3(256), 0, gw.stream, tab, gw.q_stage.get(), (uint32_t)d);
   ISL_HIP(hipGetLastError());
@@ -226,27 +259,12 @@
   u.dist = gw.dist_stage;
   u.count = gw.count_stage;
   u.mode = StreamMode::OWN;
+  u.entry = isl_lean::Entry::GROUP_MEMBER;
   ISL_TRY(search_enqueue(idx, gw, u));
-  ScatterParams sp{};
-  sp.tab = tab;
-  sp.ids = gw.ids_stage;
-  sp.dist = gw.dist_stage;
-  sp.count = gw.count_stage;
-  sp.status = gw.status;
-  sp.ctr = gw.ctr;
-  sp.redo = gw.redo;
-  sp.plog = reinterpret_cast<const uint2*>(gw.plog.get());
-  sp.ticket = gw.ticket;
-  sp.h_head = gw.h_head;
-  sp.scratch = gw.grp_scratch;
-  sp.k = (uint32_t)k;
-  sp.ef = cg.ef;
-  sp.plog_cap = cg.plog_cap;
-  hipLaunchKernelGGL(group_scatter_kernel, dim3(kScatterBlocks, nm), dim3(256), 0, gw.stream, sp);
-  ISL_HIP(hipGetLastError());
-  gw.ticket_clean = true;
-  ISL_HIP(hipEventRecord(gw.ev_done, gw.stream));
-  return ISL_OK;
+  gw.grp_members = nm;
+  gw.grp_plog_cap = cg.plog_cap;
+  if (gw.lean) idx->lean_calls.fetch_add(nm, std::memory_order_relaxed);
+  return scatter(gw, gw.lean);
 }
 
 isl_status enqueue_group(const isl_index* idx, isl::GroupState& g, const isl_group::Launch& L) {
@@ -268,6 +286,8 @@
     ws.grp_offset = mb.offset;
     ws.grp_ready = gw.ev_done;
     ws.grp_allocs = gw.alloc_events - mark;
+    ws.lean = false;
+    ws.lean_exact = false;
     ws.enqueued = true;
     ws.nq_inflight = mb.nq;
     ws.k_inflight = L.key.k;
@@ -329,7 +349,9 @@
   CallGeometry cg;
   ISL_TRY(call_geometry(idx, c.d, c.k, c.ef, nullptr, cg));
   ISL_TRY(ensure_lane_stream(idx, ws));
-  ISL_HIP(hipEventRecord(ws.ev_in, c.user_stream));
+  ws.ev_in_recorded = caller_stream_busy(c.user_stream);
+  if (ws.ev_in_recorded) ISL_HIP(hipEventRecord(ws.ev_in, c.user_stream));
+  else idx->events_elided.fetch_add(1, std::memory_order_relaxed);
   const uint32_t lane_no = (uint32_t)(&ws - idx->ws);
   std::lock_guard<std::mutex> lock(idx->group_mu);
   isl::GroupState& g = state_of(idx);
@@ -368,6 +390,23 @@
     return ws.grp_status;
   }
   return ISL_OK;
+}
+
+isl_status isl_lane::group_late_exact(const isl_index* idx, isl::SearchWorkspace& ws, bool* again) {
+  *again = false;
+  std::lock_guard<std::mutex> lock(idx->group_mu);
+  isl::SearchWorkspace* gw = ws.grp_launch;
+  if (!gw || !gw->lean) return ISL_OK;
+  ISL_TRY(group_followup(idx, *gw, isl_lean::Wait::HOST));
+  *again = gw->lean_exact;
+  return ISL_OK;
+}
+
+isl_status isl_lane::group_stream_ready(const isl_index* idx, isl::SearchWorkspace& ws) {
+  std::lock_guard<std::mutex> lock(idx->group_mu);
+  if (isl::SearchWorkspace* gw = ws.grp_launch) return gw->lean ? group_followup(idx, *gw, isl_lean::Wait::STREAM) : ISL_OK;
+  bool added = false;
+  return lean_followup(idx, ws, isl_lean::Wait::STREAM, &added);
 }
 
 void isl_lane::group_after_wait(const isl_index* idx, isl::SearchWorkspace& ws) {
diff --git a/islands_amd/csrc/search_internal.hpp b/islands_amd/csrc/search_internal.hpp
--- a/islands_amd/csrc/search_internal.hpp
+++ b/islands_amd/csrc/search_internal.hpp
@@ -1,6 +1,7 @@
 #pragma once
 
 #include "common.hpp"
+#include "lean_launch_plan.hpp"
 
 namespace isl_lane __attribute__((visibility("hidden"))) {
 
@@ -16,6 +17,7 @@
   StreamMode mode = StreamMode::OWN;
   bool two_level = false;
   float ratio = 0.0f;
+  isl_lean::Entry entry = isl_lean::Entry::DEVICE_SYNC;
 };
 inline hipStream_t call_stream(const isl::SearchWorkspace& ws, const SearchCall& c) {
   return c.mode == StreamMode::USER ? c.user_stream : ws.stream;
@@ -30,6 +32,7 @@
   uint32_t retry = 0;
   uint32_t window_scale = 1;
   bool tables_built = false;
+  bool exact_pass = false;
 };
 
 isl_status ensure_lane_stream(const isl_index* idx, isl::SearchWorkspace& ws);
@@ -42,6 +45,8 @@
 isl_status search_finish(const isl_index* idx, isl::SearchWorkspace& ws, uint32_t* misses = nullptr,
                          bool defer_statuses = false);
 isl_status search_statuses(isl::SearchWorkspace& ws, uint64_t nq);
+bool caller_stream_busy(hipStream_t user_stream);
+isl_status lean_followup(const isl_index* idx, isl::SearchWorkspace& ws, isl_lean::Wait wait, bool* added);
 isl_status search_sync(const isl_index* idx, isl::SearchWorkspace& ws, const SearchCall& c);
 
 isl_status prepare_recompute(isl::SearchWorkspace& ws, uint64_t nq, uint64_t state_words_per_query);
@@ -53,6 +58,8 @@
 isl_status group_arrive(const isl_index* idx, isl::SearchWorkspace& ws, const SearchCall& c);
 void group_pump(const isl_index* idx);
 isl_status group_before_wait(const isl_index* idx, isl::SearchWorkspace& ws);
+isl_status group_late_exact(const isl_index* idx, isl::SearchWorkspace& ws, bool* again);
+isl_status group_stream_ready(const isl_index* idx, isl::SearchWorkspace& ws);
 void group_after_wait(const isl_index* idx, isl::SearchWorkspace& ws);
 isl_status group_prepare(const isl_index* idx, uint64_t max_nq, uint64_t max_ef, uint64_t max_k, int32_t lanes,
                          uint32_t ovf_waves, uint32_t plog_cap);
diff --git a/islands_amd/csrc/search_kernels.hip.h b/islands_amd/csrc/search_kernels.hip.h
--- a/islands_amd/csrc/search_kernels.hip.h
+++ b/islands_amd/csrc/search_kernels.hip.h
@@ -21,6 +21,7 @@
   uint64_t num_nodes;
   const void* emb;
   uint32_t emb_bf16;
+  uint32_t lean_grid;
   const float* norm2;
   uint64_t nvec;
   uint64_t stride;
@@ -39,7 +40,7 @@
   uint32_t* ctr;
   uint32_t* ticket;
   uint32_t* redo;
-  uint32_t* replay;
+  const uint64_t* lean;
   uint64_t* prof;
   uint64_t* tline;
   uint2* plog;
@@ -93,6 +94,9 @@
   uint32_t pref_cap;
 };
 
+constexpr uint32_t kTicketWords = 16;
+constexpr uint32_t kTicketDone = 15;
+
 constexpr uint32_t KEY_MAX = 0xFFFFFFFFu;
 
 __device__ __forceinline__ float key_to_dist(uint32_t k) {
@@ -518,6 +522,50 @@
   }
 }
 
+template <typename T>
+__device__ __forceinline__ T late_arg(uint32_t offset) {
+  asm volatile("" : "+s"(offset));
+  const char __attribute__((address_space(4)))* args =
+      (const char __attribute__((address_space(4)))*)__builtin_amdgcn_kernarg_segment_ptr();
+  return *(const T __attribute__((address_space(4)))*)(args + offset);
+}
+
+constexpr bool lean_kernel(int S, int metric, bool bf16, bool wide, bool resume, bool qh) {
+  return !resume && !qh && !(bf16 && !wide && ((S == 8 && metric == ISL_METRIC_COSINE) ||
+                                               (S == 1 && (metric == ISL_METRIC_DOT || metric == ISL_METRIC_MANHATTAN))));
+}
+
+__device__ __forceinline__ void lean_launch_done() {
+  const uint64_t* const lean = late_arg<const uint64_t*>((uint32_t)offsetof(SearchParams, lean));
+  if (!lean) return;
+  uint32_t* const ticket = late_arg<uint32_t*>((uint32_t)offsetof(SearchParams, ticket));
+  const uint32_t workgroups = late_arg<uint32_t>((uint32_t)offsetof(SearchParams, lean_grid));
+  const uint32_t lane = threadIdx.x;
+  uint32_t last = 0;
+  __threadfence();
+  if (lane == 0) last = atomicAdd(&ticket[kTicketDone], 1u) == workgroups - 1 ? 1u : 0u;
+  if (!uni(last)) return;
+  __threadfence();
+  uint32_t* const m_status = reinterpret_cast<uint32_t*>(lean[0]);
+  uint32_t* const m_ctr = reinterpret_cast<uint32_t*>(lean[1]);
+  uint32_t* const m_head = reinterpret_cast<uint32_t*>(lean[2]);
+  if (m_status) {
+    const uint32_t nq = late_arg<uint32_t>((uint32_t)offsetof(SearchParams, nq));
+    const uint32_t* const status = late_arg<const uint32_t*>((uint32_t)offsetof(SearchParams, status));
+    const uint4* const ctr = late_arg<const uint4*>((uint32_t)offsetof(SearchParams, ctr));
+    for (uint32_t i = lane; i < nq; i += 64) {
+      m_status[i] = status[i];
+      reinterpret_cast<uint4*>(m_ctr)[i] = ctr[i];
+    }
+  }
+  if (lane < kTicketWords) {
+    const uint32_t v = __hip_atomic_load(&ticket[lane], __ATOMIC_RELAXED, __HIP_MEMORY_SCOPE_AGENT);
+    m_head[lane] = v;
+    const uint32_t redo = (uint32_t)__shfl((int)v, 1);
+    if (redo == 0) __hip_atomic_store(&ticket[lane], 0u, __ATOMIC_RELAXED, __HIP_MEMORY_SCOPE_AGENT);
+  }
+}
+
 template <int S, int METRIC_API, typename ROWT, bool WIDE, bool RESUME = false, bool QH = false>
 __global__ __launch_bounds__(64) __attribute__((amdgpu_waves_per_eu(3))) void leann_search_fast(SearchParams p) {
   static_assert(!QH || (sizeof(ROWT) == 2 && !RESUME), "the bf16 query operand goes with bf16 rows");
@@ -920,6 +968,7 @@
     }
     wave_sync();
   }
+  if constexpr (lean_kernel(S, METRIC_API, sizeof(ROWT) == 2, WIDE, RESUME, QH)) lean_launch_done();
 }
 
 
```

Result: slower. 1.582 million queries/s (-1.3%).
